# kuleshov-group/PlantCaduceus

Measured on NVIDIA B200. Metric: variants scored/sec, higher is better.
Workload: dtype bf16

## Files before the change

plantcaduceus_b200/csrc/common.cuh:

```cuda
#pragma once

#include <cuda.h>
#include <cuda_bf16.h>
#include <cuda_runtime.h>
#include <stdint.h>

#ifndef __CUDA_ARCH_FEAT_SM100_ALL
#endif

namespace pcad {

typedef __nv_bfloat16 bf16;

template <typename Kernel>
inline cudaError_t ensure_dynamic_smem(Kernel kernel, int bytes, unsigned long long& done) {
  int dev = 0;
  cudaError_t e = cudaGetDevice(&dev);
  if (e != cudaSuccess) return e;
  const unsigned long long bit = 1ull << (dev & 63);
  if (done & bit) return cudaSuccess;
  e = cudaFuncSetAttribute(kernel, cudaFuncAttributeMaxDynamicSharedMemorySize, bytes);
  if (e == cudaSuccess) done |= bit;
  return e;
}

constexpr float kLog2e = 1.4426950408889634f;
constexpr float kLn2 = 0.6931471805599453f;

template <typename T> struct ActT;
template <> struct ActT<bf16> {
  static __device__ __forceinline__ float to_f(bf16 v) { return __bfloat162float(v); }
  static __device__ __forceinline__ bf16 from_f(float v) { return __float2bfloat16_rn(v); }
};
template <> struct ActT<float> {
  static __device__ __forceinline__ float to_f(float v) { return v; }
  static __device__ __forceinline__ float from_f(float v) { return v; }
};

template <typename T> struct Vec16 { static constexpr int N = 16 / sizeof(T); };

template <typename T>
__device__ __forceinline__ void load16(const T* p, float (&out)[16 / sizeof(T)]) {
  uint4 raw = *reinterpret_cast<const uint4*>(p);
  if constexpr (sizeof(T) == 2) {
    const uint32_t w[4] = {raw.x, raw.y, raw.z, raw.w};
#pragma unroll
    for (int i = 0; i < 4; ++i) {
      out[2 * i] = __uint_as_float(w[i] << 16);
      out[2 * i + 1] = __uint_as_float(w[i] & 0xffff0000u);
    }
  } else {
    out[0] = __uint_as_float(raw.x); out[1] = __uint_as_float(raw.y);
    out[2] = __uint_as_float(raw.z); out[3] = __uint_as_float(raw.w);
  }
}

__device__ __forceinline__ uint32_t pack_bf16x2(float lo, float hi) {
  __nv_bfloat162 v = __floats2bfloat162_rn(lo, hi);
  return *reinterpret_cast<uint32_t*>(&v);
}

template <typename T>
__device__ __forceinline__ void store16(T* p, const float (&v)[16 / sizeof(T)]) {
  uint4 raw;
  if constexpr (sizeof(T) == 2) {
    raw.x = pack_bf16x2(v[0], v[1]); raw.y = pack_bf16x2(v[2], v[3]);
    raw.z = pack_bf16x2(v[4], v[5]); raw.w = pack_bf16x2(v[6], v[7]);
  } else {
    raw.x = __float_as_uint(v[0]); raw.y = __float_as_uint(v[1]);
    raw.z = __float_as_uint(v[2]); raw.w = __float_as_uint(v[3]);
  }
  *reinterpret_cast<uint4*>(p) = raw;
}

__device__ __forceinline__ float ex2_approx(float x) {
  float y;
  asm("ex2.approx.ftz.f32 %0, %1;" : "=f"(y) : "f"(x));
  return y;
}
__device__ __forceinline__ float lg2_approx(float x) {
  float y;
  asm("lg2.approx.ftz.f32 %0, %1;" : "=f"(y) : "f"(x));
  return y;
}
__device__ __forceinline__ float rcp_approx(float x) {
  float y;
  asm("rcp.approx.ftz.f32 %0, %1;" : "=f"(y) : "f"(x));
  return y;
}

template <bool PRECISE>
__device__ __forceinline__ float silu(float x) {
  if constexpr (PRECISE) {
    return x / (1.0f + expf(-x));
  } else {
    return x * rcp_approx(1.0f + ex2_approx(-x * kLog2e));
  }
}

template <bool PRECISE>
__device__ __forceinline__ float softplus(float x) {
  if constexpr (PRECISE) {
    return x > 20.0f ? x : log1pf(expf(x));
  } else {
    float sp = lg2_approx(1.0f + ex2_approx(x * kLog2e)) * kLn2;
    return x > 20.0f ? x : sp;
  }
}

typedef unsigned long long f32x2;
__device__ __forceinline__ f32x2 pack2(float lo, float hi) {
  f32x2 r;
  asm("mov.b64 %0, {%1, %2};" : "=l"(r) : "f"(lo), "f"(hi));
  return r;
}
__device__ __forceinline__ void unpack2(f32x2 v, float& lo, float& hi) {
  asm("mov.b64 {%0, %1}, %2;" : "=f"(lo), "=f"(hi) : "l"(v));
}
__device__ __forceinline__ f32x2 fma2(f32x2 a, f32x2 b, f32x2 c) {
  f32x2 r;
  asm("fma.rn.f32x2 %0, %1, %2, %3;" : "=l"(r) : "l"(a), "l"(b), "l"(c));
  return r;
}
__device__ __forceinline__ f32x2 mul2(f32x2 a, f32x2 b) {
  f32x2 r;
  asm("mul.rn.f32x2 %0, %1, %2;" : "=l"(r) : "l"(a), "l"(b));
  return r;
}
__device__ __forceinline__ f32x2 add2(f32x2 a, f32x2 b) {
  f32x2 r;
  asm("add.rn.f32x2 %0, %1, %2;" : "=l"(r) : "l"(a), "l"(b));
  return r;
}

__device__ __forceinline__ f32x2 exp2_poly2(f32x2 x2) {
  float x0, x1;
  unpack2(x2, x0, x1);
  x0 = fmaxf(x0, -126.0f);
  x1 = fmaxf(x1, -126.0f);
  x2 = pack2(x0, x1);
  const f32x2 magic = pack2(12582912.0f, 12582912.0f);
  const f32x2 r2 = add2(x2, magic);
  const f32x2 n2 = add2(r2, pack2(-12582912.0f, -12582912.0f));
  const f32x2 f2 = fma2(n2, pack2(-1.0f, -1.0f), x2);
  f32x2 p = fma2(pack2(0.009582849219441414f, 0.009582849219441414f), f2, pack2(0.05590642988681793f, 0.05590642988681793f));
  p = fma2(p, f2, pack2(0.24024099111557007f, 0.24024099111557007f));
  p = fma2(p, f2, pack2(0.6931241750717163f, 0.6931241750717163f));
  p = fma2(p, f2, pack2(1.0f, 1.0f));
  float p0, p1, r0, r1;
  unpack2(p, p0, p1);
  unpack2(r2, r0, r1);
  p0 = __int_as_float(__float_as_int(p0) + (__float_as_int(r0) << 23));
  p1 = __int_as_float(__float_as_int(p1) + (__float_as_int(r1) << 23));
  return pack2(p0, p1);
}

#ifndef PCAD_POLY_DEG
#define PCAD_POLY_DEG 4
#endif
__device__ __forceinline__ f32x2 exp2_prod_poly2(f32x2 d2, f32x2 a2) {
  const f32x2 magic = pack2(12582912.0f, 12582912.0f);
  const f32x2 r2 = fma2(d2, a2, magic);
  const f32x2 nn2 = fma2(r2, pack2(-1.0f, -1.0f), magic);
  const f32x2 f2 = fma2(d2, a2, nn2);
#if PCAD_POLY_DEG == 3
  f32x2 p = fma2(pack2(0.055009059607982635f, 0.055009059607982635f), f2, pack2(0.2422109693288803f, 0.2422109693288803f));
  p = fma2(p, f2, pack2(0.6932829022407532f, 0.6932829022407532f));
#else
  f32x2 p = fma2(pack2(0.009582576341927052f, 0.009582576341927052f), f2, pack2(0.05590682849287987f, 0.05590682849287987f));
  p = fma2(p, f2, pack2(0.24024106562137604f, 0.24024106562137604f));
  p = fma2(p, f2, pack2(0.6931241154670715f, 0.6931241154670715f));
#endif
  p = fma2(p, f2, pack2(1.0f, 1.0f));
  float p0, p1, r0, r1;
  unpack2(p, p0, p1);
  unpack2(r2, r0, r1);
  p0 = __int_as_float(__float_as_int(p0) + (__float_as_int(r0) << 23));
  p1 = __int_as_float(__float_as_int(p1) + (__float_as_int(r1) << 23));
  return pack2(p0, p1);
}

__device__ __forceinline__ float warp_sum(float v) {
#pragma unroll
  for (int o = 16; o > 0; o >>= 1) v += __shfl_xor_sync(0xffffffffu, v, o);
  return v;
}

__device__ __forceinline__ uint32_t smem_u32(const void* p) {
  return static_cast<uint32_t>(__cvta_generic_to_shared(p));
}

__device__ __forceinline__ void cp_async16(void* smem_dst, const void* gsrc, int src_bytes) {
  asm volatile("cp.async.cg.shared.global [%0], [%1], 16, %2;\n" ::"r"(smem_u32(smem_dst)), "l"(gsrc), "r"(src_bytes));
}
__device__ __forceinline__ void cp_async_commit() { asm volatile("cp.async.commit_group;\n" ::); }
template <int N>
__device__ __forceinline__ void cp_async_wait() { asm volatile("cp.async.wait_group %0;\n" ::"n"(N)); }

__device__ __forceinline__ void mbar_init(uint64_t* bar, uint32_t count) {
  asm volatile("mbarrier.init.shared::cta.b64 [%0], %1;\n" ::"r"(smem_u32(bar)), "r"(count));
}
__device__ __forceinline__ void fence_mbar_init() { asm volatile("fence.mbarrier_init.release.cluster;\n" ::); }
__device__ __forceinline__ void fence_proxy_async_smem() { asm volatile("fence.proxy.async.shared::cta;\n" ::); }

__device__ __forceinline__ void mbar_arrive_expect_tx(uint64_t* bar, uint32_t bytes) {
  asm volatile("mbarrier.arrive.expect_tx.shared::cta.b64 _, [%0], %1;\n" ::"r"(smem_u32(bar)), "r"(bytes) : "memory");
}
__device__ __forceinline__ void mbar_arrive(uint64_t* bar) {
  asm volatile("mbarrier.arrive.shared::cta.b64 _, [%0];\n" ::"r"(smem_u32(bar)) : "memory");
}
__device__ __forceinline__ bool mbar_try_wait(uint64_t* bar, uint32_t parity) {
  uint32_t ok;
  asm volatile(
      "{\n\t.reg .pred P1;\n\t"
      "mbarrier.try_wait.parity.shared::cta.b64 P1, [%1], %2;\n\t"
      "selp.b32 %0, 1, 0, P1;\n\t}\n"
      : "=r"(ok)
      : "r"(smem_u32(bar)), "r"(parity)
      : "memory");
  return ok != 0;
}
__device__ __forceinline__ void mbar_wait(uint64_t* bar, uint32_t parity) {
  while (!mbar_try_wait(bar, parity)) {
  }
}

__device__ __forceinline__ void mbar_wait_or_trap(uint64_t* bar, uint32_t parity) {
  for (uint32_t i = 0; i < (1u << 28); ++i)
    if (mbar_try_wait(bar, parity)) return;
  asm volatile("trap;");
}

__device__ __forceinline__ bool elect_one() {
  uint32_t pred;
  asm volatile(
      "{\n\t.reg .b32 rx;\n\t.reg .pred px;\n\t"
      "elect.sync rx|px, 0xffffffff;\n\t"
      "selp.b32 %0, 1, 0, px;\n\t}\n"
      : "=r"(pred));
  return pred != 0;
}

__device__ __forceinline__ void tma_prefetch_desc(const CUtensorMap* m) {
  asm volatile("prefetch.tensormap [%0];\n" ::"l"(reinterpret_cast<uint64_t>(m)) : "memory");
}
__device__ __forceinline__ void tma_load_2d(void* smem_dst, const CUtensorMap* m, uint64_t* bar, int c0, int c1) {
  asm volatile(
      "cp.async.bulk.tensor.2d.shared::cluster.global.mbarrier::complete_tx::bytes [%0], [%1, {%3, %4}], [%2];\n" ::"r"(
          smem_u32(smem_dst)),
      "l"(reinterpret_cast<uint64_t>(m)), "r"(smem_u32(bar)), "r"(c0), "r"(c1)
      : "memory");
}
__device__ __forceinline__ void tma_load_3d(void* smem_dst, const CUtensorMap* m, uint64_t* bar, int c0, int c1, int c2) {
  asm volatile(
      "cp.async.bulk.tensor.3d.shared::cluster.global.mbarrier::complete_tx::bytes [%0], [%1, {%3, %4, %5}], [%2];\n" ::"r"(
          smem_u32(smem_dst)),
      "l"(reinterpret_cast<uint64_t>(m)), "r"(smem_u32(bar)), "r"(c0), "r"(c1), "r"(c2)
      : "memory");
}
__device__ __forceinline__ void tma_prefetch_l2_3d(const CUtensorMap* m, int c0, int c1, int c2) {
  asm volatile("cp.async.bulk.prefetch.tensor.3d.L2.global [%0, {%1, %2, %3}];\n" ::"l"(reinterpret_cast<uint64_t>(m)), "r"(c0),
               "r"(c1), "r"(c2)
               : "memory");
}
__device__ __forceinline__ void tma_store_2d(const CUtensorMap* m, const void* smem_src, int c0, int c1) {
  asm volatile("cp.async.bulk.tensor.2d.global.shared::cta.bulk_group [%0, {%2, %3}], [%1];\n" ::"l"(
                   reinterpret_cast<uint64_t>(m)),
               "r"(smem_u32(smem_src)), "r"(c0), "r"(c1)
               : "memory");
}
__device__ __forceinline__ void tma_store_commit() { asm volatile("cp.async.bulk.commit_group;\n" ::: "memory"); }
template <int N>
__device__ __forceinline__ void tma_store_wait_read() {
  asm volatile("cp.async.bulk.wait_group.read %0;\n" ::"n"(N) : "memory");
}
template <int N>
__device__ __forceinline__ void tma_store_wait() {
  asm volatile("cp.async.bulk.wait_group %0;\n" ::"n"(N) : "memory");
}

template <int COLS>
__device__ __forceinline__ void tmem_alloc(uint32_t* smem_result) {
  asm volatile("tcgen05.alloc.cta_group::1.sync.aligned.shared::cta.b32 [%0], %1;\n" ::"r"(smem_u32(smem_result)), "n"(COLS)
               : "memory");
}
__device__ __forceinline__ void tmem_relinquish() {
  asm volatile("tcgen05.relinquish_alloc_permit.cta_group::1.sync.aligned;\n" ::: "memory");
}
template <int COLS>
__device__ __forceinline__ void tmem_dealloc(uint32_t taddr) {
  asm volatile("tcgen05.dealloc.cta_group::1.sync.aligned.b32 %0, %1;\n" ::"r"(taddr), "n"(COLS) : "memory");
}
__device__ __forceinline__ void tc_fence_before() { asm volatile("tcgen05.fence::before_thread_sync;\n" ::: "memory"); }
__device__ __forceinline__ void tc_fence_after() { asm volatile("tcgen05.fence::after_thread_sync;\n" ::: "memory"); }

__device__ __forceinline__ void umma_bf16_ss(uint32_t tmem_d, uint64_t desc_a, uint64_t desc_b, uint32_t idesc,
                                             uint32_t accumulate) {
  asm volatile(
      "{\n\t.reg .pred p;\n\t"
      "setp.ne.b32 p, %4, 0;\n\t"
      "tcgen05.mma.cta_group::1.kind::f16 [%0], %1, %2, %3, p;\n\t}\n" ::"r"(tmem_d),
      "l"(desc_a), "l"(desc_b), "r"(idesc), "r"(accumulate)
      : "memory");
}
__device__ __forceinline__ void umma_bf16_ss_k64_commit(uint32_t tmem_d, uint64_t desc_a, uint64_t desc_b, uint32_t idesc,
                                                        int ksteps, uint64_t* bar) {
  asm volatile(
      "{\n\t.reg .pred pz, po, p1, p2, p3;\n\t.reg .b64 a1, b1, a2, b2, a3, b3;\n\t"
      "setp.ne.b32 pz, 0, 0;\n\t"
      "setp.eq.b32 po, 0, 0;\n\t"
      "setp.gt.s32 p1, %4, 1;\n\t"
      "setp.gt.s32 p2, %4, 2;\n\t"
      "setp.gt.s32 p3, %4, 3;\n\t"
      "add.s64 a1, %1, 2;\n\tadd.s64 b1, %2, 2;\n\t"
      "add.s64 a2, %1, 4;\n\tadd.s64 b2, %2, 4;\n\t"
      "add.s64 a3, %1, 6;\n\tadd.s64 b3, %2, 6;\n\t"
      "tcgen05.mma.cta_group::1.kind::f16 [%0], %1, %2, %3, pz;\n\t"
      "@p1 tcgen05.mma.cta_group::1.kind::f16 [%0], a1, b1, %3, po;\n\t"
      "@p2 tcgen05.mma.cta_group::1.kind::f16 [%0], a2, b2, %3, po;\n\t"
      "@p3 tcgen05.mma.cta_group::1.kind::f16 [%0], a3, b3, %3, po;\n\t"
      "tcgen05.commit.cta_group::1.mbarrier::arrive::one.shared::cluster.b64 [%5];\n\t}\n" ::"r"(tmem_d),
      "l"(desc_a), "l"(desc_b), "r"(idesc), "r"(ksteps), "r"(smem_u32(bar))
      : "memory");
}
__device__ __forceinline__ void umma_commit(uint64_t* bar) {
  asm volatile("tcgen05.commit.cta_group::1.mbarrier::arrive::one.shared::cluster.b64 [%0];\n" ::"r"(smem_u32(bar))
               : "memory");
}
__device__ __forceinline__ void tmem_ld_32x32b_x32(uint32_t taddr, uint32_t (&r)[32]) {
  asm volatile(
      "tcgen05.ld.sync.aligned.32x32b.x32.b32 "
      "{%0, %1, %2, %3, %4, %5, %6, %7, %8, %9, %10, %11, %12, %13, %14, %15, "
      "%16, %17, %18, %19, %20, %21, %22, %23, %24, %25, %26, %27, %28, %29, %30, %31}, [%32];\n"
      : "=r"(r[0]), "=r"(r[1]), "=r"(r[2]), "=r"(r[3]), "=r"(r[4]), "=r"(r[5]), "=r"(r[6]), "=r"(r[7]), "=r"(r[8]),
        "=r"(r[9]), "=r"(r[10]), "=r"(r[11]), "=r"(r[12]), "=r"(r[13]), "=r"(r[14]), "=r"(r[15]), "=r"(r[16]),
        "=r"(r[17]), "=r"(r[18]), "=r"(r[19]), "=r"(r[20]), "=r"(r[21]), "=r"(r[22]), "=r"(r[23]), "=r"(r[24]),
        "=r"(r[25]), "=r"(r[26]), "=r"(r[27]), "=r"(r[28]), "=r"(r[29]), "=r"(r[30]), "=r"(r[31])
      : "r"(taddr)
      : "memory");
}
__device__ __forceinline__ void tmem_ld_32x32b_x16(uint32_t taddr, uint32_t (&r)[16]) {
  asm volatile(
      "tcgen05.ld.sync.aligned.32x32b.x16.b32 "
      "{%0, %1, %2, %3, %4, %5, %6, %7, %8, %9, %10, %11, %12, %13, %14, %15}, [%16];\n"
      : "=r"(r[0]), "=r"(r[1]), "=r"(r[2]), "=r"(r[3]), "=r"(r[4]), "=r"(r[5]), "=r"(r[6]), "=r"(r[7]), "=r"(r[8]),
        "=r"(r[9]), "=r"(r[10]), "=r"(r[11]), "=r"(r[12]), "=r"(r[13]), "=r"(r[14]), "=r"(r[15])
      : "r"(taddr)
      : "memory");
}
__device__ __forceinline__ uint32_t tmem_ld_32x32b_x1(uint32_t taddr) {
  uint32_t r;
  asm volatile("tcgen05.ld.sync.aligned.32x32b.x1.b32 {%0}, [%1];\n" : "=r"(r) : "r"(taddr) : "memory");
  return r;
}
__device__ __forceinline__ void tmem_ld_wait() { asm volatile("tcgen05.wait::ld.sync.aligned;\n" ::: "memory"); }

__device__ __forceinline__ uint32_t cluster_ctarank() {
  uint32_t r;
  asm volatile("mov.u32 %0, %%cluster_ctarank;\n" : "=r"(r));
  return r;
}
__device__ __forceinline__ void cluster_sync_all() {
  asm volatile("barrier.cluster.arrive.release.aligned;\n" ::: "memory");
  asm volatile("barrier.cluster.wait.acquire.aligned;\n" ::: "memory");
}
constexpr uint32_t kPeerBitMask = 0xFEFFFFFFu;
__device__ __forceinline__ void tma_load_2d_cg2(void* smem_dst, const CUtensorMap* m, uint64_t* bar, int c0, int c1) {
  asm volatile(
      "cp.async.bulk.tensor.2d.cta_group::2.shared::cluster.global.mbarrier::complete_tx::bytes [%0], [%1, {%3, %4}], [%2];\n" ::"r"(
          smem_u32(smem_dst)),
      "l"(reinterpret_cast<uint64_t>(m)), "r"(smem_u32(bar) & kPeerBitMask), "r"(c0), "r"(c1)
      : "memory");
}
template <int COLS>
__device__ __forceinline__ void tmem_alloc_cg2(uint32_t* smem_result) {
  asm volatile("tcgen05.alloc.cta_group::2.sync.aligned.shared::cta.b32 [%0], %1;\n" ::"r"(smem_u32(smem_result)), "n"(COLS)
               : "memory");
}
__device__ __forceinline__ void tmem_relinquish_cg2() {
  asm volatile("tcgen05.relinquish_alloc_permit.cta_group::2.sync.aligned;\n" ::: "memory");
}
template <int COLS>
__device__ __forceinline__ void tmem_dealloc_cg2(uint32_t taddr) {
  asm volatile("tcgen05.dealloc.cta_group::2.sync.aligned.b32 %0, %1;\n" ::"r"(taddr), "n"(COLS) : "memory");
}
__device__ __forceinline__ void umma_bf16_ss_cg2(uint32_t tmem_d, uint64_t desc_a, uint64_t desc_b, uint32_t idesc,
                                                 uint32_t accumulate) {
  const uint32_t zero = 0;
  asm volatile(
      "{\n\t.reg .pred p;\n\t"
      "setp.ne.b32 p, %4, 0;\n\t"
      "tcgen05.mma.cta_group::2.kind::f16 [%0], %1, %2, %3, {%5, %5, %5, %5, %5, %5, %5, %5}, p;\n\t}\n" ::"r"(tmem_d),
      "l"(desc_a), "l"(desc_b), "r"(idesc), "r"(accumulate), "r"(zero)
      : "memory");
}
__device__ __forceinline__ void umma_commit_cg2(uint64_t* bar) {
  const uint16_t mask = 3;
  asm volatile("tcgen05.commit.cta_group::2.mbarrier::arrive::one.shared::cluster.multicast::cluster.b64 [%0], %1;\n" ::"r"(
                   smem_u32(bar)),
               "h"(mask)
               : "memory");
}
__device__ __forceinline__ void mbar_arrive_leader(uint64_t* bar) {
  asm volatile("mbarrier.arrive.release.cluster.shared::cluster.b64 _, [%0];\n" ::"r"(smem_u32(bar) & kPeerBitMask) : "memory");
}

__device__ __forceinline__ uint64_t make_smem_desc_sw128(uint32_t smem_addr) {
  uint64_t desc = 0;
  desc |= static_cast<uint64_t>((smem_addr & 0x3FFFFu) >> 4);
  desc |= static_cast<uint64_t>(1) << 16;
  desc |= static_cast<uint64_t>(1024 >> 4) << 32;
  desc |= static_cast<uint64_t>(1) << 46;
  desc |= static_cast<uint64_t>(2) << 61;
  return desc;
}

__host__ __device__ constexpr uint32_t make_idesc_bf16(int M, int N) {
  return (1u << 4)
         | (1u << 7)
         | (1u << 10)
         | (0u << 15) | (0u << 16)
         | (static_cast<uint32_t>(N >> 3) << 17)
         | (static_cast<uint32_t>(M >> 4) << 24);
}

typedef CUresult (*PFN_encodeTiled)(CUtensorMap*, CUtensorMapDataType, cuuint32_t, void*, const cuuint64_t*,
                                    const cuuint64_t*, const cuuint32_t*, const cuuint32_t*, CUtensorMapInterleave,
                                    CUtensorMapSwizzle, CUtensorMapL2promotion, CUtensorMapFloatOOBfill);

inline PFN_encodeTiled get_encode_tiled() {
  static PFN_encodeTiled fn = nullptr;
  if (!fn) {
    void* p = nullptr;
    cudaDriverEntryPointQueryResult qres;
    if (cudaGetDriverEntryPoint("cuTensorMapEncodeTiled", &p, cudaEnableDefault, &qres) == cudaSuccess &&
        qres == cudaDriverEntryPointSuccess)
      fn = reinterpret_cast<PFN_encodeTiled>(p);
  }
  return fn;
}


inline bool make_tmap_3d(CUtensorMap* map, bool f32, const void* base, long long n0, long long n1, long long n2,
                         long long ld, int box0, int box1, bool swizzle128 = false) {
  PFN_encodeTiled enc = get_encode_tiled();
  if (!enc) return false;
  const cuuint64_t es = f32 ? 4 : 2;
  cuuint64_t gdim[3] = {static_cast<cuuint64_t>(n0), static_cast<cuuint64_t>(n1), static_cast<cuuint64_t>(n2)};
  cuuint64_t gstride[2] = {static_cast<cuuint64_t>(ld) * es, static_cast<cuuint64_t>(ld) * es * static_cast<cuuint64_t>(n1)};
  cuuint32_t box[3] = {static_cast<cuuint32_t>(box0), static_cast<cuuint32_t>(box1), 1};
  cuuint32_t estr[3] = {1, 1, 1};
  CUresult r = enc(map, f32 ? CU_TENSOR_MAP_DATA_TYPE_FLOAT32 : CU_TENSOR_MAP_DATA_TYPE_BFLOAT16, 3,
                   const_cast<void*>(base), gdim, gstride, box, estr, CU_TENSOR_MAP_INTERLEAVE_NONE,
                   swizzle128 ? CU_TENSOR_MAP_SWIZZLE_128B : CU_TENSOR_MAP_SWIZZLE_NONE, CU_TENSOR_MAP_L2_PROMOTION_L2_256B,
                   CU_TENSOR_MAP_FLOAT_OOB_FILL_NONE);
  return r == CUDA_SUCCESS;
}

}
```

plantcaduceus_b200/csrc/pcad.cu:

```cuda
#include "../../include/pcad.h"

#include <math.h>
#include <stdarg.h>
#include <stdio.h>
#include <stdlib.h>
#include <string.h>

#include <map>
#include <string>
#include <vector>

#include "common.cuh"
#include "elementwise.cuh"
#include "gemm_simt.cuh"
#include "gemm_tcgen05.cuh"
#include "scan.cuh"
#include "ssd.cuh"

using namespace pcad;

namespace {

char g_create_error[512] = "";

struct DirWeights {
  float* conv_w = nullptr;
  float* conv_b = nullptr;
  void* x_proj = nullptr;
  void* dt_proj = nullptr;
  float* dt_bias = nullptr;
  float* A = nullptr;
  float* D = nullptr;
  float* gnorm_w = nullptr;
  bool has[8] = {false, false, false, false, false, false, false, false};
};

struct LayerWeights {
  void* in_proj = nullptr;
  void* in_proj_s = nullptr;
  void* out_proj = nullptr;
  float* norm_w = nullptr;
  DirWeights dir[2];
  bool has_in = false, has_out = false, has_norm = false;
};

struct Workspace {
  int B = 0, L = 0;
  size_t bytes = 0;
  uint8_t* base = nullptr;
  uint8_t* ids = nullptr;
  void* hid = nullptr;
  void* resid = nullptr;
  void* normed = nullptr;
  void* xz = nullptr;
  void* xc[2] = {nullptr, nullptr};
  void* dbc[2] = {nullptr, nullptr};
  void* delta[2] = {nullptr, nullptr};
  void* y = nullptr;
  float* sumsq[2] = {nullptr, nullptr};
  float* seg_state = nullptr;
  float* seg_sumd = nullptr;
  float* bcf = nullptr;
  uint8_t* ascii = nullptr;
  float* logits4 = nullptr;
  int* pos = nullptr;
  int* pos0 = nullptr;
};

}

struct pcad_handle {
  pcad_config cfg;
  int device = 0;
  int num_sms = 148;
  int d = 0, E = 0, N = 16, R = 0, RP = 0, V = 8;
  bool m2 = false;
  int ssd_impl = 0;
  int H = 0, CD = 0, DIP = 0, DIPP = 0;
  bool f32 = false;
  bool fuse_dt = false;
  bool bc_f32 = true;
  bool bc_f32_force = false;
  bool fuse_norm = false;
  size_t act_size = 2;
  bool finalized = false;
  char err[512] = "";
  std::vector<LayerWeights> layers;
  void* emb = nullptr;
  float* head_w = nullptr;
  float* norm_f = nullptr;
  bool has_emb = false, has_head = false, has_norm_f = false;
  uint8_t* comp_dev = nullptr;
  uint8_t* lut_dev = nullptr;
  int* sel_dev = nullptr;
  int* bad_flag = nullptr;
  volatile int* bad_flag_host = nullptr;
  int mask_id = 1;
  int acgt[4] = {3, 4, 5, 6};
  Workspace ws;
  std::vector<void*> allocs;
  struct ScoreGraph { int B, L, token_idx; bool seen_only; cudaGraphExec_t exec; int64_t launches; };
  std::vector<ScoreGraph> graphs;
  bool prune_last = true;
  bool last_pruned = false;
  bool time_parallel = true;
  bool use_graphs = true;
  cudaStream_t gstream = nullptr;
  cudaEvent_t g_in = nullptr, g_out = nullptr;
  long long graph_max_tokens = 65536;
  bool profiling = false;
  std::vector<std::pair<int, std::pair<cudaEvent_t, cudaEvent_t>>> prof_events;
  std::vector<cudaEvent_t> event_pool;
  float prof_ms[PCAD_ST_COUNT];
  int64_t prof_launches[PCAD_ST_COUNT];
  int64_t launch_count = 0;
};

namespace {

int fail(pcad_handle* h, int code, const char* fmt, ...) {
  va_list ap;
  va_start(ap, fmt);
  char* dst = h ? h->err : g_create_error;
  vsnprintf(dst, 512, fmt, ap);
  va_end(ap);
  return code;
}

#define CUDA_TRY(h, expr)                                                                          \
  do {                                                                                             \
    cudaError_t _e = (expr);                                                                       \
    if (_e != cudaSuccess)                                                                         \
      return fail((h), PCAD_ERR_CUDA, "%s failed: %s (%s:%d)", #expr, cudaGetErrorString(_e), __FILE__, __LINE__); \
  } while (0)

template <typename T>
int dev_alloc(pcad_handle* h, T** p, size_t count) {
  void* q = nullptr;
  cudaError_t e = cudaMalloc(&q, count * sizeof(T) > 0 ? count * sizeof(T) : 16);
  if (e != cudaSuccess) return fail(h, PCAD_ERR_NOMEM, "cudaMalloc(%zu) failed: %s", count * sizeof(T), cudaGetErrorString(e));
  h->allocs.push_back(q);
  *p = static_cast<T*>(q);
  return PCAD_OK;
}

template <typename SrcT, typename DstT>
__global__ void convert_kernel(const SrcT* __restrict__ src, DstT* __restrict__ dst, long long n) {
  const long long i = static_cast<long long>(blockIdx.x) * blockDim.x + threadIdx.x;
  if (i >= n) return;
  float v;
  if constexpr (sizeof(SrcT) == 2) v = __bfloat162float(src[i]); else v = src[i];
  if constexpr (sizeof(DstT) == 2) dst[i] = __float2bfloat16_rn(v); else dst[i] = v;
}
__global__ void half_to_float_kernel(const __half* __restrict__ src, float* __restrict__ dst, long long n) {
  const long long i = static_cast<long long>(blockIdx.x) * blockDim.x + threadIdx.x;
  if (i < n) dst[i] = __half2float(src[i]);
}
__global__ void scale_columns_kernel(const bf16* __restrict__ W, const float* __restrict__ w, bf16* __restrict__ out,
                                     long long rows, int cols) {
  const long long i = static_cast<long long>(blockIdx.x) * blockDim.x + threadIdx.x;
  if (i >= rows * cols) return;
  out[i] = __float2bfloat16_rn(__bfloat162float(W[i]) * w[i % cols]);
}
__global__ void row_sumsq_kernel(const bf16* __restrict__ x, float* __restrict__ ss, long long rows, int d, int parts) {
  const int lane = threadIdx.x & 31;
  const long long row = static_cast<long long>(blockIdx.x) * (blockDim.x >> 5) + (threadIdx.x >> 5);
  if (row >= rows) return;
  float acc = 0.f;
  for (int j = lane * 8; j < d; j += 256) {
    float v[8];
    load16<bf16>(x + row * d + j, v);
#pragma unroll
    for (int k = 0; k < 8; ++k) acc = fmaf(v[k], v[k], acc);
  }
  acc = warp_sum(acc);
  if (lane < parts) ss[row * parts + lane] = lane == 0 ? acc : 0.f;
}
__global__ void neg_exp_kernel(float* __restrict__ a, long long n) {
  const long long i = static_cast<long long>(blockIdx.x) * blockDim.x + threadIdx.x;
  if (i < n) a[i] = -expf(a[i]);
}

int ingest(pcad_handle* h, const void* src, int src_dtype, void* dst, bool dst_f32, long long n) {
  const size_t src_size = (src_dtype == PCAD_F32) ? 4 : 2;
  void* stage = nullptr;
  CUDA_TRY(h, cudaMalloc(&stage, n * src_size));
  cudaError_t e = cudaMemcpy(stage, src, n * src_size, cudaMemcpyDefault);
  if (e != cudaSuccess) { cudaFree(stage); return fail(h, PCAD_ERR_CUDA, "weight copy failed: %s", cudaGetErrorString(e)); }
  float* f32_tmp = nullptr;
  const void* s = stage;
  int s_dtype = src_dtype;
  const int threads = 256;
  const unsigned blocks = static_cast<unsigned>((n + threads - 1) / threads);
  if (src_dtype == PCAD_F16) {
    e = cudaMalloc(reinterpret_cast<void**>(&f32_tmp), n * 4);
    if (e != cudaSuccess) { cudaFree(stage); return fail(h, PCAD_ERR_NOMEM, "cudaMalloc failed"); }
    half_to_float_kernel<<<blocks, threads>>>(static_cast<const __half*>(stage), f32_tmp, n);
    s = f32_tmp;
    s_dtype = PCAD_F32;
  }
  if (s_dtype == PCAD_F32) {
    if (dst_f32) convert_kernel<float, float><<<blocks, threads>>>(static_cast<const float*>(s), static_cast<float*>(dst), n);
    else convert_kernel<float, bf16><<<blocks, threads>>>(static_cast<const float*>(s), static_cast<bf16*>(dst), n);
  } else {
    if (dst_f32) convert_kernel<bf16, float><<<blocks, threads>>>(static_cast<const bf16*>(s), static_cast<float*>(dst), n);
    else convert_kernel<bf16, bf16><<<blocks, threads>>>(static_cast<const bf16*>(s), static_cast<bf16*>(dst), n);
  }
  e = cudaDeviceSynchronize();
  cudaFree(stage);
  if (f32_tmp) cudaFree(f32_tmp);
  if (e != cudaSuccess) return fail(h, PCAD_ERR_CUDA, "weight conversion failed: %s", cudaGetErrorString(e));
  return PCAD_OK;
}

bool shape_is(const int64_t* shape, int ndim, std::initializer_list<int64_t> want) {
  std::vector<int64_t> a, b;
  for (int i = 0; i < ndim; ++i) if (shape[i] != 1) a.push_back(shape[i]);
  for (int64_t w : want) if (w != 1) b.push_back(w);
  return a == b;
}

struct StageTimer {
  pcad_handle* h;
  cudaStream_t st;
  int stage;
  cudaEvent_t a = nullptr, b = nullptr;
  StageTimer(pcad_handle* h_, cudaStream_t st_, int stage_, int launches = 1) : h(h_), st(st_), stage(stage_) {
    h->launch_count += launches;
    if (!h->profiling) return;
    h->prof_launches[stage] += launches;
    auto get = [&]() {
      cudaEvent_t ev;
      if (!h->event_pool.empty()) { ev = h->event_pool.back(); h->event_pool.pop_back(); }
      else cudaEventCreate(&ev);
      return ev;
    };
    a = get(); b = get();
    cudaEventRecord(a, st);
  }
  ~StageTimer() {
    if (!a) return;
    cudaEventRecord(b, st);
    h->prof_events.push_back({stage, {a, b}});
  }
};

bool gemm_cta_pair_enabled() {
  static int v = -1;
  if (v < 0) {
    const char* e = getenv("PCAD_GEMM_2CTA");
    v = (e && e[0] == '0') ? 0 : 1;
  }
  return v == 1;
}

int op_linear(pcad_handle* h, const void* A, const void* W, void* C, long long M, int N, int K, long long lda,
              long long ldw, long long ldc, bool f32, int num_sms, cudaStream_t st, int epi = kEpiPlain,
              const EpiParams& ep = EpiParams()) {
  if (f32) {
    if (epi != kEpiPlain) return fail(h, PCAD_ERR_INVALID, "fused GEMM epilogues exist for bf16 only");
    CUDA_TRY(h, gemm_f32_simt(static_cast<const float*>(A), static_cast<const float*>(W), static_cast<float*>(C), M, N, K, lda, ldw, ldc, st));
  } else {
    const char* why = nullptr;
    cudaError_t e = gemm_bf16_tcgen05(static_cast<const bf16*>(A), static_cast<const bf16*>(W), static_cast<bf16*>(C), M, N, K, lda, ldw, ldc, num_sms, st, &why, epi, ep, gemm_cta_pair_enabled());
    if (e != cudaSuccess) return fail(h, why ? PCAD_ERR_INVALID : PCAD_ERR_CUDA, "%s", why ? why : cudaGetErrorString(e));
  }
  return PCAD_OK;
}

template <typename T, typename RT>
int launch_norm_t(pcad_handle* h, const void* x, const void* res_in, const float* w, void* y, void* res_out,
                  long long rows, int d, float eps, cudaStream_t st) {
  const int nvec = d / 8;
  const int ch = (nvec + 31) / 32;
  const int warps = 8;
  const unsigned blocks = static_cast<unsigned>((rows + warps - 1) / warps);
#define NORM_CASE(CHV)                                                                                          \
  add_rmsnorm_kernel<T, RT, CHV><<<blocks, warps * 32, 0, st>>>(static_cast<const T*>(x), static_cast<const RT*>(res_in), w, \
                                                               static_cast<T*>(y), static_cast<RT*>(res_out), rows, d, eps)
  if (ch <= 1) NORM_CASE(1);
  else if (ch <= 2) NORM_CASE(2);
  else if (ch <= 4) NORM_CASE(4);
  else if (ch <= 8) NORM_CASE(8);
  else return fail(h, PCAD_ERR_INVALID, "add_rmsnorm: d=%d too large (max 2048)", d);
#undef NORM_CASE
  CUDA_TRY(h, cudaGetLastError());
  return PCAD_OK;
}

int op_add_rmsnorm(pcad_handle* h, const void* x, const void* res_in, const float* w, void* y, void* res_out,
                   long long rows, int d, float eps, bool f32, bool res_f32, cudaStream_t st) {
  if (d % 8) return fail(h, PCAD_ERR_INVALID, "add_rmsnorm: d must be a multiple of 8");
  if (rows <= 0) return PCAD_OK;
  if (f32) return launch_norm_t<float, float>(h, x, res_in, w, y, res_out, rows, d, eps, st);
  if (res_f32) return launch_norm_t<bf16, float>(h, x, res_in, w, y, res_out, rows, d, eps, st);
  return launch_norm_t<bf16, bf16>(h, x, res_in, w, y, res_out, rows, d, eps, st);
}

int op_conv(pcad_handle* h, const void* x, long long ldx, const float* w_f, const float* b_f, const float* w_r,
            const float* b_r, void* out_f, void* out_r, int S, int L, int E, bool f32, cudaStream_t st) {
  if (E % 4) return fail(h, PCAD_ERR_INVALID, "conv: E must be a multiple of 4");
  if (S <= 0 || L <= 0) return PCAD_OK;
  const int cpt = f32 ? 4 : 2;
  dim3 grid((E / cpt + 127) / 128, (L + kConvTT - 1) / kConvTT, S);
  if (f32) conv_silu_kernel<float, true, 4><<<grid, 128, 0, st>>>(static_cast<const float*>(x), ldx, w_f, b_f, w_r, b_r, static_cast<float*>(out_f), static_cast<float*>(out_r), L, E);
  else conv_silu_kernel<bf16, false, 2><<<grid, 128, 0, st>>>(static_cast<const bf16*>(x), ldx, w_f, b_f, w_r, b_r, static_cast<bf16*>(out_f), static_cast<bf16*>(out_r), L, E);
  CUDA_TRY(h, cudaGetLastError());
  return PCAD_OK;
}

int op_biscan(pcad_handle* h, const void* u_f, const void* delta_f, const void* bc_f, const void* u_r,
              const void* delta_r, const void* bc_r, long long ldbc, int bc_off, const void* z, long long ldz,
              const float* A_f, const float* D_f, const float* bias_f, const float* A_r, const float* D_r,
              const float* bias_r, void* y, int S, int L, int E, bool f32, cudaStream_t st,
              const void* wdt_f = nullptr, const void* wdt_r = nullptr, long long ldw = 0, int R = 0, int segments = 1,
              float* seg_state = nullptr, float* seg_sumd = nullptr, int Lrun = 0, float* bcf = nullptr) {
  const int vec = f32 ? 4 : 8;
  if (E % vec || ldbc % vec || bc_off % vec || ldz % vec)
    return fail(h, PCAD_ERR_INVALID, "biscan: E, ldbc, bc_off, ldz must be multiples of %d elements", vec);
  if (S <= 0 || L <= 0) return PCAD_OK;
  if (S > 65535) return fail(h, PCAD_ERR_INVALID, "biscan: at most 65535 sequences per call");
  cudaError_t e;
#define PCAD_SCAN_ARGS(TT)                                                                                           \
  static_cast<const TT*>(u_f), static_cast<const TT*>(delta_f), static_cast<const TT*>(bc_f), static_cast<const TT*>(u_r), \
      static_cast<const TT*>(delta_r), static_cast<const TT*>(bc_r), ldbc, bc_off, static_cast<const TT*>(z), ldz, A_f, D_f, \
      bias_f, A_r, D_r, bias_r, static_cast<TT*>(y), S, L, E
  const bool fused_dt = wdt_f != nullptr || wdt_r != nullptr;
  const float* bcf_f = nullptr;
  const float* bcf_r = nullptr;
  if (bcf && !f32 && !fused_dt) {
    const long long rows = static_cast<long long>(S) * L;
    bc_to_f32_kernel<<<static_cast<unsigned>((rows * 8 + 255) / 256), 256, 0, st>>>(static_cast<const bf16*>(bc_f), static_cast<const bf16*>(bc_r),
                                                                                  ldbc, bc_off, bcf, rows);
    CUDA_TRY(h, cudaGetLastError());
    bcf_f = bcf;
    bcf_r = bcf + rows * 2 * kScanN;
  }
  if (segments > 1) {
    if (fused_dt || !seg_state || !seg_sumd || L % segments || static_cast<long long>(S) * segments > 65535)
      return fail(h, PCAD_ERR_INVALID, "biscan: the time-parallel scan needs L %% segments == 0, S * segments <= 65535 and its state buffers");
    if (f32) e = launch_biscan_time_parallel<float, true>(PCAD_SCAN_ARGS(float), segments, seg_state, seg_sumd, st);
    else e = launch_biscan_time_parallel<bf16, false>(PCAD_SCAN_ARGS(bf16), segments, seg_state, seg_sumd, st, bcf_f, bcf_r);
    CUDA_TRY(h, e);
    return PCAD_OK;
  }
  if (fused_dt) {
    if (f32 || !wdt_f || !wdt_r || ldbc < kScanDtK || R <= 0 || R > kScanDtK || ldw < R || ldw % 8)
      return fail(h, PCAD_ERR_INVALID, "biscan: the in-kernel dt_proj needs bf16, both weights (R <= 64, row pitch a multiple of 8) and ldbc >= 64");
    e = launch_biscan<bf16, false, kScanFusedDt>(PCAD_SCAN_ARGS(bf16), st, static_cast<const bf16*>(wdt_f), static_cast<const bf16*>(wdt_r),
                                                 ldw, R, nullptr, Lrun);
  } else if (f32) {
    e = launch_biscan<float, true, kScanPlain>(PCAD_SCAN_ARGS(float), st, nullptr, nullptr, 0, 0, nullptr, Lrun);
  } else if (bcf_f) {
    e = launch_biscan<bf16, false, kScanBcF32>(PCAD_SCAN_ARGS(bf16), st, nullptr, nullptr, 0, 0, nullptr, Lrun, bcf_f, bcf_r);
  } else {
    e = launch_biscan<bf16, false, kScanPlain>(PCAD_SCAN_ARGS(bf16), st, nullptr, nullptr, 0, 0, nullptr, Lrun);
  }
#undef PCAD_SCAN_ARGS
  CUDA_TRY(h, e);
  return PCAD_OK;
}

size_t align_up(size_t v, size_t a) { return (v + a - 1) / a * a; }
constexpr size_t kSegStateBytes = 16u << 20;

size_t workspace_layout(const pcad_handle* h, int B, int L, Workspace* ws) {
  const size_t T = 2ull * B * L;
  const size_t a = h->act_size;
  const size_t rs = h->f32 ? 4 : (h->cfg.residual_in_fp32 ? 4 : 2);
  size_t off = 0;
  auto take = [&](size_t bytes) { size_t o = off; off = align_up(off + bytes, 1024); return o; };
  const size_t o_ids = take(static_cast<size_t>(B) * L);
  const size_t o_hid = take(T * h->d * a);
  const size_t o_res = take(T * h->d * rs);
  const size_t o_nrm = take(T * h->d * a);
  const size_t w_xz = h->m2 ? h->DIPP : 2 * h->E, w_xc = h->m2 ? h->CD : h->E, w_dbc = h->m2 ? 0 : h->RP;
  const size_t o_xz = take(T * w_xz * a);
  const size_t o_xc0 = take(T * w_xc * a), o_xc1 = take(T * w_xc * a);
  const size_t o_dbc0 = take(T * w_dbc * a), o_dbc1 = take(T * w_dbc * a);
  const size_t o_dl0 = take(T * h->E * a), o_dl1 = take(T * h->E * a);
  const size_t o_y = take(T * h->E * a);
  const size_t ss_parts = static_cast<size_t>(gemm_sumsq_parts(h->d));
  const size_t o_ss0 = take(T * ss_parts * sizeof(float)), o_ss1 = take(T * ss_parts * sizeof(float));
  const size_t o_segs = take(h->m2 ? 0 : kSegStateBytes), o_segd = take(h->m2 ? 0 : kSegStateBytes / 16);
  const size_t o_bcf = take((h->m2 || h->f32) ? 0 : T * 2 * 2 * kScanN * sizeof(float));
  const size_t o_ascii = take(static_cast<size_t>(B) * L);
  const size_t o_l4 = take(static_cast<size_t>(B) * 4 * sizeof(float));
  const size_t o_pos = take(static_cast<size_t>(B) * sizeof(int));
  const size_t o_pos0 = take(static_cast<size_t>(B) * sizeof(int));
  if (ws && ws->base) {
    uint8_t* p = ws->base;
    ws->ids = p + o_ids; ws->hid = p + o_hid; ws->resid = p + o_res; ws->normed = p + o_nrm; ws->xz = p + o_xz;
    ws->xc[0] = p + o_xc0; ws->xc[1] = p + o_xc1; ws->dbc[0] = p + o_dbc0; ws->dbc[1] = p + o_dbc1;
    ws->delta[0] = p + o_dl0; ws->delta[1] = p + o_dl1; ws->y = p + o_y;
    ws->sumsq[0] = reinterpret_cast<float*>(p + o_ss0); ws->sumsq[1] = reinterpret_cast<float*>(p + o_ss1);
    ws->seg_state = reinterpret_cast<float*>(p + o_segs); ws->seg_sumd = reinterpret_cast<float*>(p + o_segd);
    ws->bcf = (h->m2 || h->f32) ? nullptr : reinterpret_cast<float*>(p + o_bcf);
    ws->ascii = p + o_ascii; ws->logits4 = reinterpret_cast<float*>(p + o_l4); ws->pos = reinterpret_cast<int*>(p + o_pos);
    ws->pos0 = reinterpret_cast<int*>(p + o_pos0);
  }
  return off;
}

void clear_graphs(pcad_handle* h) {
  for (auto& g : h->graphs)
    if (g.exec) cudaGraphExecDestroy(g.exec);
  h->graphs.clear();
}

int ensure_workspace(pcad_handle* h, int B, int L) {
  Workspace& ws = h->ws;
  const size_t need = workspace_layout(h, B, L, nullptr);
  if (ws.base == nullptr || need > ws.bytes) {
    clear_graphs(h);
    if (ws.base) { cudaDeviceSynchronize(); cudaFree(ws.base); ws.base = nullptr; ws.bytes = 0; }
    void* p = nullptr;
    cudaError_t e = cudaMalloc(&p, need);
    if (e != cudaSuccess) return fail(h, PCAD_ERR_NOMEM, "workspace cudaMalloc(%zu bytes) for B=%d L=%d failed: %s", need, B, L, cudaGetErrorString(e));
    ws.base = static_cast<uint8_t*>(p);
    ws.bytes = need;
  }
  ws.B = B; ws.L = L;
  workspace_layout(h, B, L, &ws);
  return PCAD_OK;
}

int op_ssd_scan(pcad_handle* h, const void* xbc_f, const void* xbc_r, long long ld_xbc, const void* dt_raw, long long ld_dt,
                const float* A_f, const float* D_f, const float* bias_f, const float* A_r, const float* D_r, const float* bias_r,
                void* y_f, void* y_r, int S, int L, int H, bool f32, int impl, cudaStream_t st) {
  const bool sequential = impl == 1;
  if (S <= 0 || L <= 0) return PCAD_OK;
  if (H <= 0 || S > 65535) return fail(h, PCAD_ERR_INVALID, "ssd_scan: need H > 0 and at most 65535 sequences per call");
  cudaError_t e;
  if (f32) {
    e = launch_ssd_seq<float>(static_cast<const float*>(xbc_f), static_cast<const float*>(xbc_r), ld_xbc, static_cast<const float*>(dt_raw),
                              ld_dt, A_f, D_f, bias_f, A_r, D_r, bias_r, static_cast<float*>(y_f), static_cast<float*>(y_r), S, L, H, st);
  } else if (sequential) {
    e = launch_ssd_seq<bf16>(static_cast<const bf16*>(xbc_f), static_cast<const bf16*>(xbc_r), ld_xbc, static_cast<const bf16*>(dt_raw),
                             ld_dt, A_f, D_f, bias_f, A_r, D_r, bias_r, static_cast<bf16*>(y_f), static_cast<bf16*>(y_r), S, L, H, st);
  } else {
    if ((H & 1) || (ld_xbc % 8) || (reinterpret_cast<uintptr_t>(xbc_f) & 15) || (reinterpret_cast<uintptr_t>(xbc_r) & 15) ||
        (reinterpret_cast<uintptr_t>(y_f) & 15) || (reinterpret_cast<uintptr_t>(y_r) & 15))
      return fail(h, PCAD_ERR_INVALID, "ssd_scan: the tensor-core kernel needs an even head count, 16-byte aligned tensors and ld_xbc %% 8 == 0");
    e = launch_ssd_tc(static_cast<const bf16*>(xbc_f), static_cast<const bf16*>(xbc_r), ld_xbc, static_cast<const bf16*>(dt_raw), ld_dt,
                      A_f, D_f, bias_f, A_r, D_r, bias_r, static_cast<bf16*>(y_f), static_cast<bf16*>(y_r), S, L, H, st);
  }
  CUDA_TRY(h, e);
  return PCAD_OK;
}

int op_gated_norm_sum(pcad_handle* h, const void* y_f, const void* y_r, const void* z, long long ldz, const float* w_f,
                      const float* w_r, void* out, long long rows, int E, float eps, bool f32, cudaStream_t st) {
  if (rows <= 0) return PCAD_OK;
  const int vec = f32 ? 4 : 8;
  if (E % vec || ldz % vec) return fail(h, PCAD_ERR_INVALID, "gated_norm_sum: E and ldz must be multiples of %d", vec);
  const unsigned blocks = static_cast<unsigned>((rows + 7) / 8);
  if (!f32 && E <= 256 * 12) {
    const int ch = (E + 255) / 256;
#define GN_CASE(CHV)                                                                                                        \
  gated_norm_sum_regs_kernel<CHV><<<blocks, 256, 0, st>>>(static_cast<const bf16*>(y_f), static_cast<const bf16*>(y_r),        \
                                                          static_cast<const bf16*>(z), ldz, w_f, w_r, static_cast<bf16*>(out), rows, E, eps)
    if (ch <= 1) GN_CASE(1);
    else if (ch <= 2) GN_CASE(2);
    else if (ch <= 3) GN_CASE(3);
    else if (ch <= 4) GN_CASE(4);
    else if (ch <= 6) GN_CASE(6);
    else if (ch <= 8) GN_CASE(8);
    else GN_CASE(12);
#undef GN_CASE
    CUDA_TRY(h, cudaGetLastError());
    return PCAD_OK;
  }
  if (f32) gated_norm_sum_kernel<float, true><<<blocks, 256, 0, st>>>(static_cast<const float*>(y_f), static_cast<const float*>(y_r), static_cast<const float*>(z), ldz, w_f, w_r, static_cast<float*>(out), rows, E, eps);
  else gated_norm_sum_kernel<bf16, false><<<blocks, 256, 0, st>>>(static_cast<const bf16*>(y_f), static_cast<const bf16*>(y_r), static_cast<const bf16*>(z), ldz, w_f, w_r, static_cast<bf16*>(out), rows, E, eps);
  CUDA_TRY(h, cudaGetLastError());
  return PCAD_OK;
}

int run_mixer_m2(pcad_handle* h, LayerWeights& lw, int S, int L, cudaStream_t st) {
  Workspace& ws = h->ws;
  const long long T = static_cast<long long>(S) * L;
  const int E = h->E, CD = h->CD, H = h->H;
  const bool f32 = h->f32;
  const size_t a = h->act_size;
  uint8_t* zx = static_cast<uint8_t*>(ws.xz);
  int rc;
  {
    StageTimer tm(h, st, PCAD_ST_CONV);
    rc = op_conv(h, zx + static_cast<size_t>(E) * a, h->DIPP, lw.dir[0].conv_w, lw.dir[0].conv_b, lw.dir[1].conv_w, lw.dir[1].conv_b,
                 ws.xc[0], ws.xc[1], S, L, CD, f32, st);
    if (rc) return rc;
  }
  {
    StageTimer tm(h, st, PCAD_ST_SCAN);
    rc = op_ssd_scan(h, ws.xc[0], ws.xc[1], CD, zx + static_cast<size_t>(E + CD) * a, h->DIPP, lw.dir[0].A, lw.dir[0].D, lw.dir[0].dt_bias,
                     lw.dir[1].A, lw.dir[1].D, lw.dir[1].dt_bias, ws.delta[0], ws.delta[1], S, L, H, f32, h->ssd_impl, st);
    if (rc) return rc;
  }
  {
    StageTimer tm(h, st, PCAD_ST_GNORM);
    rc = op_gated_norm_sum(h, ws.delta[0], ws.delta[1], zx, h->DIPP, lw.dir[0].gnorm_w, lw.dir[1].gnorm_w, ws.y, T, E, 1e-5f, f32, st);
    if (rc) return rc;
  }
  return PCAD_OK;
}

__global__ void gather_rows_kernel(const uint4* __restrict__ src, uint4* __restrict__ dst, int S, int B, int L, int idx, int vec_per_row) {
  const long long gid = static_cast<long long>(blockIdx.x) * blockDim.x + threadIdx.x;
  if (gid >= static_cast<long long>(S) * vec_per_row) return;
  const int s = static_cast<int>(gid / vec_per_row), v = static_cast<int>(gid % vec_per_row);
  const int row = s < B ? idx : L - 1 - idx;
  dst[gid] = src[(static_cast<long long>(s) * L + row) * vec_per_row + v];
}

int run_backbone(pcad_handle* h, int B, int L, cudaStream_t st, int prune_idx = -1) {
  Workspace& ws = h->ws;
  const long long T = 2LL * B * L;
  const int S = 2 * B;
  const int d = h->d, E = h->E, R = h->R, RP = h->RP;
  const bool f32 = h->f32;
  const bool res_f32 = f32 || h->cfg.residual_in_fp32;
  const bool fused = h->fuse_norm;
  int cur = 0;
  h->last_pruned = false;
  const int parts = gemm_sumsq_parts(d);
  const int n_in = h->m2 ? h->DIP : 2 * E;
  const long long ld_in = h->m2 ? h->DIPP : 2 * E;
  {
    StageTimer tm(h, st, PCAD_ST_EMBED, fused ? 2 : 1);
    const long long total = T * (d / 8);
    const unsigned blocks = static_cast<unsigned>((total + 255) / 256);
    if (f32) embed_kernel<float><<<blocks, 256, 0, st>>>(ws.ids, static_cast<const float*>(h->emb), static_cast<float*>(ws.hid), B, L, d, h->comp_dev);
    else embed_kernel<bf16><<<blocks, 256, 0, st>>>(ws.ids, static_cast<const bf16*>(h->emb), static_cast<bf16*>(fused ? ws.resid : ws.hid), B, L, d, h->comp_dev);
    if (fused) row_sumsq_kernel<<<static_cast<unsigned>((T + 7) / 8), 256, 0, st>>>(static_cast<const bf16*>(ws.resid), ws.sumsq[cur], T, d, parts);
    CUDA_TRY(h, cudaGetLastError());
  }
  for (int li = 0; li < h->cfg.n_layer; ++li) {
    LayerWeights& lw = h->layers[li];
    int rc;
    bool pruned = false;
    if (!fused) {
      StageTimer tm(h, st, PCAD_ST_NORM);
      rc = op_add_rmsnorm(h, ws.hid, li == 0 ? nullptr : ws.resid, lw.norm_w, ws.normed, ws.resid, T, d, h->cfg.norm_eps, f32, res_f32, st);
      if (rc) return rc;
    }
    {
      StageTimer tm(h, st, PCAD_ST_IN_PROJ);
      if (fused) {
        EpiParams ep;
        ep.sumsq_in = ws.sumsq[cur];
        ep.sumsq_parts = parts;
        ep.inv_k = 1.0f / static_cast<float>(d);
        ep.eps = h->cfg.norm_eps;
        rc = op_linear(h, ws.resid, lw.in_proj_s, ws.xz, T, n_in, d, d, d, ld_in, false, h->num_sms, st, kEpiRowScale, ep);
      } else {
        rc = op_linear(h, ws.normed, lw.in_proj, ws.xz, T, n_in, d, d, d, ld_in, f32, h->num_sms, st);
      }
      if (rc) return rc;
    }
    if (h->m2) {
      rc = run_mixer_m2(h, lw, S, L, st);
      if (rc) return rc;
    } else {
    {
      StageTimer tm(h, st, PCAD_ST_CONV);
      rc = op_conv(h, ws.xz, 2 * E, lw.dir[0].conv_w, lw.dir[0].conv_b, lw.dir[1].conv_w, lw.dir[1].conv_b, ws.xc[0], ws.xc[1], S, L, E, f32, st);
      if (rc) return rc;
    }
    int P = 1;
    if (h->time_parallel) {
      const long long ctas = static_cast<long long>((E + kScanCH - 1) / kScanCH) * S, slots = 4LL * h->num_sms;
      while (P < 32 && ctas * P * 2 <= slots && L % (P * 2) == 0 && L / (P * 2) >= 512 &&
             static_cast<size_t>(S) * P * 2 * 2 * E * kScanN * sizeof(float) <= kSegStateBytes)
        P *= 2;
    }
    const bool fuse_dt = h->fuse_dt && P == 1;
    for (int dir = 0; dir < 2; ++dir) {
      {
        StageTimer tm(h, st, PCAD_ST_X_PROJ);
        rc = op_linear(h, ws.xc[dir], lw.dir[dir].x_proj, ws.dbc[dir], T, RP, E, E, E, RP, f32, h->num_sms, st);
        if (rc) return rc;
      }
      if (!fuse_dt) {
        StageTimer tm(h, st, PCAD_ST_DT_PROJ);
        rc = op_linear(h, ws.dbc[dir], lw.dir[dir].dt_proj, ws.delta[dir], T, E, R, RP, R, E, f32, h->num_sms, st);
        if (rc) return rc;
      }
    }
    {
      StageTimer tm(h, st, PCAD_ST_SCAN);
      const uint8_t* zbase = static_cast<const uint8_t*>(ws.xz) + static_cast<size_t>(E) * h->act_size;
      pruned = prune_idx >= 0 && li == h->cfg.n_layer - 1 && P == 1 && h->prune_last && L >= 8;
      const int Lrun = pruned ? (prune_idx > L - 1 - prune_idx ? prune_idx : L - 1 - prune_idx) + 1 : 0;
      const bool use_bcf = h->bc_f32 && !f32 && (h->bc_f32_force || T >= 65536);
      if (fuse_dt)
        rc = op_biscan(h, ws.xc[0], ws.dbc[0], ws.dbc[0], ws.xc[1], ws.dbc[1], ws.dbc[1], RP, R, zbase, 2 * E,
                       lw.dir[0].A, lw.dir[0].D, lw.dir[0].dt_bias, lw.dir[1].A, lw.dir[1].D, lw.dir[1].dt_bias, ws.y, S, L, E, f32,
                       st, lw.dir[0].dt_proj, lw.dir[1].dt_proj, R, R, 1, nullptr, nullptr, Lrun);
      else {
        rc = op_biscan(h, ws.xc[0], ws.delta[0], ws.dbc[0], ws.xc[1], ws.delta[1], ws.dbc[1], RP, R, zbase, 2 * E,
                       lw.dir[0].A, lw.dir[0].D, lw.dir[0].dt_bias, lw.dir[1].A, lw.dir[1].D, lw.dir[1].dt_bias, ws.y, S, L, E, f32, st,
                       nullptr, nullptr, 0, 0, P, ws.seg_state, ws.seg_sumd, Lrun, use_bcf ? ws.bcf : nullptr);
        if (P > 1) h->launch_count += 2;
        if (use_bcf) h->launch_count += 1;
      }
      if (rc) return rc;
    }
    }
    if (pruned) {
      h->last_pruned = true;
      const size_t a = h->act_size, rs = res_f32 ? 4 : a;
      uint8_t* yc = static_cast<uint8_t*>(ws.delta[0]);
      uint8_t* rc_in = static_cast<uint8_t*>(ws.delta[1]);
      uint8_t* rc_out = rc_in + align_up(static_cast<size_t>(S) * d * 4, 1024);
      {
        StageTimer tm(h, st, PCAD_ST_MISC, 2);
        const int vy = static_cast<int>(E * a / 16), vr = static_cast<int>(d * rs / 16);
        gather_rows_kernel<<<static_cast<unsigned>((static_cast<long long>(S) * vy + 255) / 256), 256, 0, st>>>(
            static_cast<const uint4*>(ws.y), reinterpret_cast<uint4*>(yc), S, B, L, prune_idx, vy);
        if (fused || li > 0)
          gather_rows_kernel<<<static_cast<unsigned>((static_cast<long long>(S) * vr + 255) / 256), 256, 0, st>>>(
              static_cast<const uint4*>(ws.resid), reinterpret_cast<uint4*>(rc_in), S, B, L, prune_idx, vr);
        CUDA_TRY(h, cudaGetLastError());
      }
      {
        StageTimer tm(h, st, PCAD_ST_OUT_PROJ);
        if (fused) {
          EpiParams ep;
          ep.resid = reinterpret_cast<const bf16*>(rc_in);
          ep.ld_res = d;
          ep.sumsq_out = ws.sumsq[cur ^ 1];
          ep.sumsq_parts = parts;
          rc = op_linear(h, yc, lw.out_proj, rc_out, S, d, E, E, E, d, false, h->num_sms, st, kEpiResidual, ep);
        } else {
          rc = op_linear(h, yc, lw.out_proj, rc_out, S, d, E, E, E, d, f32, h->num_sms, st);
        }
        if (rc) return rc;
      }
      StageTimer tm(h, st, PCAD_ST_NORM);
      if (fused) rc = op_add_rmsnorm(h, rc_out, nullptr, h->norm_f, ws.normed, nullptr, S, d, h->cfg.norm_eps, false, false, st);
      else rc = op_add_rmsnorm(h, rc_out, li == 0 ? nullptr : rc_in, h->norm_f, ws.normed, nullptr, S, d, h->cfg.norm_eps, f32, res_f32, st);
      return rc;
    }
    {
      StageTimer tm(h, st, PCAD_ST_OUT_PROJ);
      if (fused) {
        EpiParams ep;
        ep.resid = static_cast<const bf16*>(ws.resid);
        ep.ld_res = d;
        ep.sumsq_out = ws.sumsq[cur ^ 1];
        ep.sumsq_parts = parts;
        rc = op_linear(h, ws.y, lw.out_proj, ws.resid, T, d, E, E, E, d, false, h->num_sms, st, kEpiResidual, ep);
        cur ^= 1;
      } else {
        rc = op_linear(h, ws.y, lw.out_proj, ws.hid, T, d, E, E, E, d, f32, h->num_sms, st);
      }
      if (rc) return rc;
    }
  }
  {
    StageTimer tm(h, st, PCAD_ST_NORM);
    int rc;
    if (fused) rc = op_add_rmsnorm(h, ws.resid, nullptr, h->norm_f, ws.normed, nullptr, T, d, h->cfg.norm_eps, false, false, st);
    else rc = op_add_rmsnorm(h, ws.hid, h->cfg.n_layer == 0 ? nullptr : ws.resid, h->norm_f, ws.normed, nullptr, T, d, h->cfg.norm_eps, f32, res_f32, st);
    if (rc) return rc;
  }
  return PCAD_OK;
}

int run_head(pcad_handle* h, int B, int L, const int* pos_dev, int n_pos, float* out, cudaStream_t st) {
  StageTimer tm(h, st, PCAD_ST_HEAD);
  const long long items = pos_dev ? static_cast<long long>(B) * n_pos : static_cast<long long>(B) * L;
  if (items <= 0) return PCAD_OK;
  const unsigned blocks = static_cast<unsigned>((items + 7) / 8);
  if (h->f32) lm_head_kernel<float><<<blocks, 256, 0, st>>>(static_cast<const float*>(h->ws.normed), h->head_w, h->comp_dev, pos_dev, n_pos, h->sel_dev, out, B, L, h->d);
  else lm_head_kernel<bf16><<<blocks, 256, 0, st>>>(static_cast<const bf16*>(h->ws.normed), h->head_w, h->comp_dev, pos_dev, n_pos, h->sel_dev, out, B, L, h->d);
  CUDA_TRY(h, cudaGetLastError());
  return PCAD_OK;
}

__global__ void fill_int_kernel(int* p, int n, int v) {
  const int i = blockIdx.x * blockDim.x + threadIdx.x;
  if (i < n) p[i] = v;
}

int check_call(pcad_handle* h, int B, int L) {
  if (!h) return PCAD_ERR_INVALID;
  if (!h->finalized) return fail(h, PCAD_ERR_STATE, "pcad_finalize must succeed before a forward call");
  if (B < 0 || L < 0) return fail(h, PCAD_ERR_INVALID, "negative batch or length");
  if (2LL * B > 65535) return fail(h, PCAD_ERR_INVALID, "B=%d too large for one call (max 32767)", B);
  return PCAD_OK;
}

}

extern "C" {

int pcad_abi_version(void) { return PCAD_ABI_VERSION; }

const char* pcad_last_error(const pcad_handle* h) { return h ? h->err : g_create_error; }

int pcad_create(const pcad_config* cfg, int device, pcad_handle** out) {
  if (!cfg || !out) return fail(nullptr, PCAD_ERR_INVALID, "null argument");
  *out = nullptr;
  const bool m2 = cfg->mixer == PCAD_MIXER_MAMBA2;
  if (cfg->mixer != PCAD_MIXER_MAMBA1 && !m2) return fail(nullptr, PCAD_ERR_INVALID, "unknown mixer %d", cfg->mixer);
  if (m2) {
    if (cfg->d_state != 64 || cfg->headdim != 64 || cfg->ngroups != 1)
      return fail(nullptr, PCAD_ERR_INVALID, "unsupported Mamba-2 shape d_state=%d headdim=%d ngroups=%d (engine is specialised for 64 / 64 / 1)",
                  cfg->d_state, cfg->headdim, cfg->ngroups);
    if ((cfg->expand * cfg->d_model / 64) % 2) return fail(nullptr, PCAD_ERR_INVALID, "Mamba-2 needs an even number of heads");
  } else if (cfg->d_state != 16) {
    return fail(nullptr, PCAD_ERR_INVALID, "unsupported d_state=%d (engine is specialised for 16)", cfg->d_state);
  }
  if (cfg->d_conv != 4) return fail(nullptr, PCAD_ERR_INVALID, "unsupported d_conv=%d (engine is specialised for 4)", cfg->d_conv);
  if (cfg->vocab_size != 8) return fail(nullptr, PCAD_ERR_INVALID, "unsupported vocab_size=%d (LM head is specialised for 8 rows)", cfg->vocab_size);
  if (cfg->d_model <= 0 || cfg->d_model % 128 != 0 || cfg->d_model > 2048)
    return fail(nullptr, PCAD_ERR_INVALID, "unsupported d_model=%d (need a multiple of 128, <= 2048)", cfg->d_model);
  if (cfg->expand != 2) return fail(nullptr, PCAD_ERR_INVALID, "unsupported expand=%d", cfg->expand);
  if (!m2 && (cfg->dt_rank <= 0 || cfg->dt_rank % 8 != 0)) return fail(nullptr, PCAD_ERR_INVALID, "unsupported dt_rank=%d (need a multiple of 8)", cfg->dt_rank);
  if (cfg->n_layer < 0) return fail(nullptr, PCAD_ERR_INVALID, "negative n_layer");
  if (cfg->dtype != PCAD_BF16 && cfg->dtype != PCAD_F32) return fail(nullptr, PCAD_ERR_INVALID, "dtype must be PCAD_BF16 or PCAD_F32");
  for (int i = 0; i < cfg->vocab_size; ++i)
    if (cfg->complement_map[i] < 0 || cfg->complement_map[i] >= cfg->vocab_size)
      return fail(nullptr, PCAD_ERR_INVALID, "complement_map[%d]=%d out of range", i, cfg->complement_map[i]);
  int ndev = 0;
  cudaError_t e = cudaGetDeviceCount(&ndev);
  if (e != cudaSuccess || ndev == 0)
    return fail(nullptr, PCAD_ERR_CUDA, "no CUDA device available (%s); libpcad has no CPU fallback", cudaGetErrorString(e));
  if (device < 0 || device >= ndev) return fail(nullptr, PCAD_ERR_INVALID, "device %d out of range (have %d)", device, ndev);
  e = cudaSetDevice(device);
  if (e != cudaSuccess) return fail(nullptr, PCAD_ERR_CUDA, "cudaSetDevice failed: %s", cudaGetErrorString(e));
  cudaDeviceProp prop;
  cudaGetDeviceProperties(&prop, device);
  if (prop.major != 10)
    return fail(nullptr, PCAD_ERR_CUDA, "device %d is sm_%d%d; libpcad is built for sm_100a only", device, prop.major, prop.minor);

  pcad_handle* h = new pcad_handle();
  h->cfg = *cfg;
  h->device = device;
  h->num_sms = prop.multiProcessorCount;
  h->d = cfg->d_model;
  h->E = cfg->expand * cfg->d_model;
  h->N = cfg->d_state;
  h->R = cfg->dt_rank;
  h->RP = (h->R + 2 * h->N + 15) / 16 * 16;
  h->m2 = m2;
  if (m2) {
    h->H = h->E / 64;
    h->CD = h->E + 2 * h->N;
    h->DIP = h->E + h->CD + h->H;
    h->DIPP = (h->DIP + 7) / 8 * 8;
    h->R = 0;
    h->RP = 0;
    if (const char* sq = getenv("PCAD_SSD_SEQ")) h->ssd_impl = sq[0] == '1' ? 1 : 0;
  }
  h->V = cfg->vocab_size;
  h->f32 = cfg->dtype == PCAD_F32;
  h->act_size = h->f32 ? 4 : 2;
  h->fuse_norm = !h->f32 && !cfg->residual_in_fp32;
  h->fuse_dt = false;
  if (const char* fd = getenv("PCAD_FUSED_DT"))
    h->fuse_dt = fd[0] == '1' && !m2 && !h->f32 && h->RP >= kScanDtK && h->R <= kScanDtK && (h->E % 8) == 0;
  if (const char* bq = getenv("PCAD_SCAN_BC_F32")) { h->bc_f32 = bq[0] != '0'; h->bc_f32_force = bq[0] == '1'; }
  if (const char* pl = getenv("PCAD_NO_PRUNE")) h->prune_last = pl[0] != '1';
  if (const char* tp = getenv("PCAD_NO_TIME_PARALLEL")) h->time_parallel = tp[0] != '1';
  if (const char* ng = getenv("PCAD_NO_GRAPH")) h->use_graphs = ng[0] != '1';
  if (const char* gm = getenv("PCAD_GRAPH_MAX_TOKENS")) h->graph_max_tokens = atoll(gm);
  if (const char* nf = getenv("PCAD_NO_FUSED_NORM")) { if (nf[0] == '1') h->fuse_norm = false; }
  memset(h->prof_ms, 0, sizeof(h->prof_ms));
  memset(h->prof_launches, 0, sizeof(h->prof_launches));
  h->layers.resize(cfg->n_layer);
  int rc = PCAD_OK;
  const size_t a = h->act_size;
  auto A8 = [&](void** p, size_t bytes) { uint8_t* q; int r = dev_alloc<uint8_t>(h, &q, bytes); *p = q; return r; };
  rc |= A8(&h->emb, static_cast<size_t>(h->V) * h->d * a);
  rc |= dev_alloc(h, &h->head_w, static_cast<size_t>(h->V) * h->d);
  rc |= dev_alloc(h, &h->norm_f, h->d);
  rc |= dev_alloc(h, &h->comp_dev, 16);
  rc |= dev_alloc(h, &h->lut_dev, 256);
  rc |= dev_alloc(h, &h->sel_dev, 4);
  {
    void* hp = nullptr;
    void* dp = nullptr;
    if (cudaHostAlloc(&hp, sizeof(int), cudaHostAllocMapped) != cudaSuccess || cudaHostGetDevicePointer(&dp, hp, 0) != cudaSuccess) {
      if (hp) cudaFreeHost(hp);
      rc |= fail(h, PCAD_ERR_NOMEM, "cudaHostAlloc for the id-error flag failed");
    } else {
      h->bad_flag_host = static_cast<volatile int*>(hp);
      *h->bad_flag_host = 0;
      h->bad_flag = static_cast<int*>(dp);
    }
  }
  const size_t n_in_rows = m2 ? static_cast<size_t>(h->DIP) : static_cast<size_t>(2) * h->E;
  for (auto& lw : h->layers) {
    rc |= A8(&lw.in_proj, n_in_rows * h->d * a);
    if (h->fuse_norm) rc |= A8(&lw.in_proj_s, n_in_rows * h->d * a);
    rc |= A8(&lw.out_proj, static_cast<size_t>(h->d) * h->E * a);
    rc |= dev_alloc(h, &lw.norm_w, h->d);
    for (int dir = 0; dir < 2; ++dir) {
      DirWeights& dw = lw.dir[dir];
      if (m2) {
        rc |= dev_alloc(h, &dw.conv_w, static_cast<size_t>(h->CD) * 4);
        rc |= dev_alloc(h, &dw.conv_b, h->CD);
        rc |= dev_alloc(h, &dw.dt_bias, h->H);
        rc |= dev_alloc(h, &dw.A, h->H);
        rc |= dev_alloc(h, &dw.D, h->H);
        rc |= dev_alloc(h, &dw.gnorm_w, h->E);
        continue;
      }
      rc |= dev_alloc(h, &dw.conv_w, static_cast<size_t>(h->E) * 4);
      rc |= dev_alloc(h, &dw.conv_b, h->E);
      rc |= A8(&dw.x_proj, static_cast<size_t>(h->RP) * h->E * a);
      rc |= A8(&dw.dt_proj, static_cast<size_t>(h->E) * h->R * a);
      rc |= dev_alloc(h, &dw.dt_bias, h->E);
      rc |= dev_alloc(h, &dw.A, static_cast<size_t>(h->E) * h->N);
      rc |= dev_alloc(h, &dw.D, h->E);
      if (rc == PCAD_OK) cudaMemset(dw.x_proj, 0, static_cast<size_t>(h->RP) * h->E * a);
    }
    if (rc != PCAD_OK) break;
  }
  if (rc != PCAD_OK) {
    snprintf(g_create_error, sizeof(g_create_error), "%.511s", h->err);
    pcad_destroy(h);
    return PCAD_ERR_NOMEM;
  }
  uint8_t comp8[16] = {0};
  for (int i = 0; i < h->V; ++i) comp8[i] = static_cast<uint8_t>(cfg->complement_map[i]);
  cudaMemcpy(h->comp_dev, comp8, 16, cudaMemcpyHostToDevice);
  uint8_t lut[256];
  memset(lut, 2, sizeof(lut));
  lut['a'] = lut['A'] = 3; lut['c'] = lut['C'] = 4; lut['g'] = lut['G'] = 5; lut['t'] = lut['T'] = 6;
  const int32_t acgt[4] = {3, 4, 5, 6};
  *out = h;
  return pcad_set_tokenizer(h, lut, 1, acgt);
}

void pcad_destroy(pcad_handle* h) {
  if (!h) return;
  cudaSetDevice(h->device);
  cudaDeviceSynchronize();
  for (auto& pe : h->prof_events) { cudaEventDestroy(pe.second.first); cudaEventDestroy(pe.second.second); }
  for (auto ev : h->event_pool) cudaEventDestroy(ev);
  clear_graphs(h);
  if (h->gstream) cudaStreamDestroy(h->gstream);
  if (h->g_in) cudaEventDestroy(h->g_in);
  if (h->g_out) cudaEventDestroy(h->g_out);
  if (h->ws.base) cudaFree(h->ws.base);
  if (h->bad_flag_host) cudaFreeHost(const_cast<int*>(h->bad_flag_host));
  for (void* p : h->allocs) cudaFree(p);
  delete h;
}

int pcad_set_tokenizer(pcad_handle* h, const uint8_t lut[256], int mask_id, const int32_t acgt_ids[4]) {
  if (!h || !lut || !acgt_ids) return PCAD_ERR_INVALID;
  if (mask_id < 0 || mask_id >= h->V) return fail(h, PCAD_ERR_INVALID, "mask_id %d out of range", mask_id);
  for (int i = 0; i < 256; ++i) if (lut[i] >= h->V) return fail(h, PCAD_ERR_INVALID, "lut[%d]=%d out of range", i, lut[i]);
  for (int k = 0; k < 4; ++k) if (acgt_ids[k] < 0 || acgt_ids[k] >= h->V) return fail(h, PCAD_ERR_INVALID, "acgt id out of range");
  CUDA_TRY(h, cudaSetDevice(h->device));
  CUDA_TRY(h, cudaMemcpy(h->lut_dev, lut, 256, cudaMemcpyHostToDevice));
  int sel[4] = {acgt_ids[0], acgt_ids[1], acgt_ids[2], acgt_ids[3]};
  CUDA_TRY(h, cudaMemcpy(h->sel_dev, sel, sizeof(sel), cudaMemcpyHostToDevice));
  h->mask_id = mask_id;
  for (int k = 0; k < 4; ++k) h->acgt[k] = acgt_ids[k];
  clear_graphs(h);
  return PCAD_OK;
}

int pcad_set_weight(pcad_handle* h, const char* name, const void* data, const int64_t* shape, int ndim, int src_dtype) {
  if (!h || !name || !data || !shape) return PCAD_ERR_INVALID;
  if (src_dtype != PCAD_BF16 && src_dtype != PCAD_F32 && src_dtype != PCAD_F16) return fail(h, PCAD_ERR_INVALID, "bad src_dtype for %s", name);
  CUDA_TRY(h, cudaSetDevice(h->device));
  h->finalized = false;
  clear_graphs(h);
  const int d = h->d, E = h->E, N = h->N, R = h->R, V = h->V;
  const std::string s(name);
  auto bad_shape = [&]() { return fail(h, PCAD_ERR_INVALID, "unexpected shape for %s", name); };
  if (s == "caduceus.backbone.embeddings.word_embeddings.embedding.weight") {
    if (!shape_is(shape, ndim, {V, d})) return bad_shape();
    int rc = ingest(h, data, src_dtype, h->emb, h->f32, static_cast<long long>(V) * d);
    h->has_emb = rc == PCAD_OK;
    return rc;
  }
  if (s == "lm_head.lm_head.weight") {
    if (!shape_is(shape, ndim, {V, d})) return bad_shape();
    int rc = ingest(h, data, src_dtype, h->head_w, true, static_cast<long long>(V) * d);
    h->has_head = rc == PCAD_OK;
    return rc;
  }
  if (s == "caduceus.backbone.norm_f.weight") {
    if (!shape_is(shape, ndim, {d})) return bad_shape();
    int rc = ingest(h, data, src_dtype, h->norm_f, true, d);
    h->has_norm_f = rc == PCAD_OK;
    return rc;
  }
  const std::string lp = "caduceus.backbone.layers.";
  if (s.compare(0, lp.size(), lp) != 0) return fail(h, PCAD_ERR_INVALID, "unknown weight name %s", name);
  size_t dot = s.find('.', lp.size());
  if (dot == std::string::npos) return fail(h, PCAD_ERR_INVALID, "unknown weight name %s", name);
  const int li = atoi(s.substr(lp.size(), dot - lp.size()).c_str());
  if (li < 0 || li >= h->cfg.n_layer) return fail(h, PCAD_ERR_INVALID, "layer index out of range in %s", name);
  LayerWeights& lw = h->layers[li];
  const std::string rest = s.substr(dot + 1);
  if (rest == "norm.weight") {
    if (!shape_is(shape, ndim, {d})) return bad_shape();
    int rc = ingest(h, data, src_dtype, lw.norm_w, true, d);
    lw.has_norm = rc == PCAD_OK;
    return rc;
  }
  const std::string mp = "mixer.submodule.mamba_";
  if (rest.compare(0, mp.size(), mp) != 0) return fail(h, PCAD_ERR_INVALID, "unknown weight name %s", name);
  int dir;
  if (rest.compare(mp.size(), 4, "fwd.") == 0) dir = 0;
  else if (rest.compare(mp.size(), 4, "rev.") == 0) dir = 1;
  else return fail(h, PCAD_ERR_INVALID, "unknown weight name %s", name);
  const std::string leaf = rest.substr(mp.size() + 4);
  DirWeights& dw = lw.dir[dir];
  int rc;
  const int n_in = h->m2 ? h->DIP : 2 * E;
  const int CE = h->m2 ? h->CD : E;
  const int NH = h->m2 ? h->H : E;
  if (leaf == "in_proj.weight") {
    if (!shape_is(shape, ndim, {n_in, d})) return bad_shape();
    if (dir == 1 && lw.has_in) return PCAD_OK;
    rc = ingest(h, data, src_dtype, lw.in_proj, h->f32, static_cast<long long>(n_in) * d);
    lw.has_in = rc == PCAD_OK;
  } else if (leaf == "out_proj.weight") {
    if (!shape_is(shape, ndim, {d, E})) return bad_shape();
    if (dir == 1 && lw.has_out) return PCAD_OK;
    rc = ingest(h, data, src_dtype, lw.out_proj, h->f32, static_cast<long long>(d) * E);
    lw.has_out = rc == PCAD_OK;
  } else if (leaf == "conv1d.weight") {
    if (!shape_is(shape, ndim, {CE, 4})) return bad_shape();
    rc = ingest(h, data, src_dtype, dw.conv_w, true, static_cast<long long>(CE) * 4);
    dw.has[0] = rc == PCAD_OK;
  } else if (leaf == "conv1d.bias") {
    if (!shape_is(shape, ndim, {CE})) return bad_shape();
    rc = ingest(h, data, src_dtype, dw.conv_b, true, CE);
    dw.has[1] = rc == PCAD_OK;
  } else if (leaf == "x_proj.weight" && !h->m2) {
    if (!shape_is(shape, ndim, {R + 2 * N, E})) return bad_shape();
    rc = ingest(h, data, src_dtype, dw.x_proj, h->f32, static_cast<long long>(R + 2 * N) * E);
    dw.has[2] = rc == PCAD_OK;
  } else if (leaf == "dt_proj.weight" && !h->m2) {
    if (!shape_is(shape, ndim, {E, R})) return bad_shape();
    rc = ingest(h, data, src_dtype, dw.dt_proj, h->f32, static_cast<long long>(E) * R);
    dw.has[3] = rc == PCAD_OK;
  } else if ((leaf == "dt_proj.bias" && !h->m2) || (leaf == "dt_bias" && h->m2)) {
    if (!shape_is(shape, ndim, {NH})) return bad_shape();
    rc = ingest(h, data, src_dtype, dw.dt_bias, true, NH);
    dw.has[4] = rc == PCAD_OK;
  } else if (leaf == "A_log") {
    const long long n = h->m2 ? NH : static_cast<long long>(E) * N;
    if (h->m2 ? !shape_is(shape, ndim, {NH}) : !shape_is(shape, ndim, {E, N})) return bad_shape();
    rc = ingest(h, data, src_dtype, dw.A, true, n);
    if (rc == PCAD_OK) {
      neg_exp_kernel<<<static_cast<unsigned>((n + 255) / 256), 256>>>(dw.A, n);
      CUDA_TRY(h, cudaDeviceSynchronize());
    }
    dw.has[5] = rc == PCAD_OK;
  } else if (leaf == "D") {
    if (!shape_is(shape, ndim, {NH})) return bad_shape();
    rc = ingest(h, data, src_dtype, dw.D, true, NH);
    dw.has[6] = rc == PCAD_OK;
  } else if (leaf == "norm.weight" && h->m2) {
    if (!shape_is(shape, ndim, {E})) return bad_shape();
    rc = ingest(h, data, src_dtype, dw.gnorm_w, true, E);
    dw.has[7] = rc == PCAD_OK;
  } else {
    return fail(h, PCAD_ERR_INVALID, "unknown weight name %s", name);
  }
  return rc;
}

int pcad_finalize(pcad_handle* h) {
  if (!h) return PCAD_ERR_INVALID;
  if (!h->has_emb) return fail(h, PCAD_ERR_MISSING, "missing weight: embedding");
  if (!h->has_norm_f) return fail(h, PCAD_ERR_MISSING, "missing weight: norm_f");
  if (!h->has_head) {
    const long long n = static_cast<long long>(h->V) * h->d;
    CUDA_TRY(h, cudaSetDevice(h->device));
    if (h->f32) convert_kernel<float, float><<<static_cast<unsigned>((n + 255) / 256), 256>>>(static_cast<const float*>(h->emb), h->head_w, n);
    else convert_kernel<bf16, float><<<static_cast<unsigned>((n + 255) / 256), 256>>>(static_cast<const bf16*>(h->emb), h->head_w, n);
    CUDA_TRY(h, cudaDeviceSynchronize());
    h->has_head = true;
  }
  static const char* names1[8] = {"conv1d.weight", "conv1d.bias", "x_proj.weight", "dt_proj.weight", "dt_proj.bias", "A_log", "D", nullptr};
  static const char* names2[8] = {"conv1d.weight", "conv1d.bias", nullptr, nullptr, "dt_bias", "A_log", "D", "norm.weight"};
  const char** names = h->m2 ? names2 : names1;
  for (int li = 0; li < h->cfg.n_layer; ++li) {
    const LayerWeights& lw = h->layers[li];
    if (!lw.has_in) return fail(h, PCAD_ERR_MISSING, "missing weight: layers.%d in_proj.weight", li);
    if (!lw.has_out) return fail(h, PCAD_ERR_MISSING, "missing weight: layers.%d out_proj.weight", li);
    if (!lw.has_norm) return fail(h, PCAD_ERR_MISSING, "missing weight: layers.%d norm.weight", li);
    for (int dir = 0; dir < 2; ++dir)
      for (int k = 0; k < 8; ++k)
        if (names[k] && !lw.dir[dir].has[k]) return fail(h, PCAD_ERR_MISSING, "missing weight: layers.%d mamba_%s.%s", li, dir ? "rev" : "fwd", names[k]);
  }
  if (h->fuse_norm) {
    CUDA_TRY(h, cudaSetDevice(h->device));
    const long long rows = h->m2 ? h->DIP : 2LL * h->E, n = rows * h->d;
    for (auto& lw : h->layers)
      scale_columns_kernel<<<static_cast<unsigned>((n + 255) / 256), 256>>>(static_cast<const bf16*>(lw.in_proj), lw.norm_w,
                                                                           static_cast<bf16*>(lw.in_proj_s), rows, h->d);
    CUDA_TRY(h, cudaDeviceSynchronize());
  }
  h->finalized = true;
  return PCAD_OK;
}

int pcad_workspace_bytes(pcad_handle* h, int B, int L, size_t* out) {
  if (!h || !out || B < 0 || L < 0) return PCAD_ERR_INVALID;
  *out = workspace_layout(h, B, L, nullptr);
  return PCAD_OK;
}

int pcad_tokenize(pcad_handle* h, const uint8_t* ascii_dev, int64_t n, uint8_t* ids_dev, void* stream) {
  if (!h || (n > 0 && (!ascii_dev || !ids_dev))) return PCAD_ERR_INVALID;
  if (n <= 0) return PCAD_OK;
  CUDA_TRY(h, cudaSetDevice(h->device));
  cudaStream_t st = static_cast<cudaStream_t>(stream);
  StageTimer tm(h, st, PCAD_ST_MISC);
  tokenize_kernel<<<static_cast<unsigned>((n + 255) / 256), 256, 0, st>>>(ascii_dev, ids_dev, n, h->lut_dev, 1, -1, 0);
  CUDA_TRY(h, cudaGetLastError());
  return PCAD_OK;
}

int pcad_extract_windows(pcad_handle* h, const uint8_t* chrom_dev, int64_t chrom_len, const int64_t* pos0_dev, int B, int L,
                         int token_idx, uint8_t* ascii_out_dev, void* stream) {
  if (!h || B < 0 || L <= 0 || chrom_len < 0) return PCAD_ERR_INVALID;
  if (B == 0) return PCAD_OK;
  if (!chrom_dev || !pos0_dev || !ascii_out_dev) return fail(h, PCAD_ERR_INVALID, "null argument");
  if (token_idx < 0 || token_idx >= L) return fail(h, PCAD_ERR_INVALID, "token_idx %d outside [0, %d)", token_idx, L);
  CUDA_TRY(h, cudaSetDevice(h->device));
  cudaStream_t st = static_cast<cudaStream_t>(stream);
  StageTimer tm(h, st, PCAD_ST_MISC);
  const long long n = static_cast<long long>(B) * L;
  extract_windows_kernel<<<static_cast<unsigned>((n + 255) / 256), 256, 0, st>>>(
      chrom_dev, chrom_len, reinterpret_cast<const long long*>(pos0_dev), ascii_out_dev, B, L, token_idx);
  CUDA_TRY(h, cudaGetLastError());
  return PCAD_OK;
}

namespace {
int score_core(pcad_handle* h, int B, int L, int token_idx, cudaStream_t st) {
  Workspace& ws = h->ws;
  const long long n = static_cast<long long>(B) * L;
  {
    StageTimer tm(h, st, PCAD_ST_MISC, 3);
    tokenize_kernel<<<static_cast<unsigned>((n + 255) / 256), 256, 0, st>>>(ws.ascii, ws.ids, n, h->lut_dev, L, token_idx, h->mask_id);
    fill_int_kernel<<<(B + 255) / 256, 256, 0, st>>>(ws.pos, B, token_idx);
    fill_int_kernel<<<(B + 255) / 256, 256, 0, st>>>(ws.pos0, B, 0);
    CUDA_TRY(h, cudaGetLastError());
  }
  const bool prune = h->prune_last && !h->m2 && h->cfg.n_layer > 0;
  int rc = run_backbone(h, B, L, st, prune ? token_idx : -1);
  if (rc) return rc;
  if (prune && h->last_pruned) return run_head(h, B, 1, ws.pos0, 1, ws.logits4, st);
  return run_head(h, B, L, ws.pos, 1, ws.logits4, st);
}

int score_core_graphed(pcad_handle* h, int B, int L, int token_idx, cudaStream_t st) {
  if (!h->use_graphs || h->profiling || 2LL * B * L > h->graph_max_tokens) return score_core(h, B, L, token_idx, st);
  pcad_handle::ScoreGraph* e = nullptr;
  for (auto& g : h->graphs)
    if (g.B == B && g.L == L && g.token_idx == token_idx) { e = &g; break; }
  if (!e) {
    h->graphs.push_back({B, L, token_idx, true, nullptr, 0});
    return score_core(h, B, L, token_idx, st);
  }
  if (!h->gstream) {
    if (cudaStreamCreateWithFlags(&h->gstream, cudaStreamNonBlocking) != cudaSuccess ||
        cudaEventCreateWithFlags(&h->g_in, cudaEventDisableTiming) != cudaSuccess ||
        cudaEventCreateWithFlags(&h->g_out, cudaEventDisableTiming) != cudaSuccess) {
      h->use_graphs = false;
      cudaGetLastError();
      return score_core(h, B, L, token_idx, st);
    }
  }
  if (e->seen_only) {
    const int64_t before = h->launch_count;
    cudaGraph_t graph = nullptr;
    cudaError_t ce = cudaStreamBeginCapture(h->gstream, cudaStreamCaptureModeThreadLocal);
    int rc = ce == cudaSuccess ? score_core(h, B, L, token_idx, h->gstream) : PCAD_ERR_CUDA;
    if (ce == cudaSuccess) ce = cudaStreamEndCapture(h->gstream, &graph);
    if (rc == PCAD_OK && ce == cudaSuccess && graph) ce = cudaGraphInstantiate(&e->exec, graph, 0);
    if (graph) cudaGraphDestroy(graph);
    if (rc != PCAD_OK || ce != cudaSuccess || !e->exec) {
      e->exec = nullptr;
      h->use_graphs = false;
      h->launch_count = before;
      cudaGetLastError();
      return score_core(h, B, L, token_idx, st);
    }
    e->launches = h->launch_count - before;
    h->launch_count = before;
    e->seen_only = false;
  }
  CUDA_TRY(h, cudaEventRecord(h->g_in, st));
  CUDA_TRY(h, cudaStreamWaitEvent(h->gstream, h->g_in, 0));
  CUDA_TRY(h, cudaGraphLaunch(e->exec, h->gstream));
  CUDA_TRY(h, cudaEventRecord(h->g_out, h->gstream));
  CUDA_TRY(h, cudaStreamWaitEvent(st, h->g_out, 0));
  h->launch_count += e->launches;
  return PCAD_OK;
}
}

int pcad_score_windows_dev(pcad_handle* h, const uint8_t* ascii_dev, int B, int L, int token_idx, float* logits4_dev, void* stream) {
  int rc = check_call(h, B, L);
  if (rc) return rc;
  if (B == 0 || L == 0) return PCAD_OK;
  if (!ascii_dev || !logits4_dev) return fail(h, PCAD_ERR_INVALID, "null argument");
  if (token_idx < 0 || token_idx >= L) return fail(h, PCAD_ERR_INVALID, "token_idx %d outside [0, %d)", token_idx, L);
  CUDA_TRY(h, cudaSetDevice(h->device));
  cudaStream_t st = static_cast<cudaStream_t>(stream);
  rc = ensure_workspace(h, B, L);
  if (rc) return rc;
  Workspace& ws = h->ws;
  const size_t n = static_cast<size_t>(B) * L;
  CUDA_TRY(h, cudaMemcpyAsync(ws.ascii, ascii_dev, n, cudaMemcpyDeviceToDevice, st));
  rc = score_core_graphed(h, B, L, token_idx, st);
  if (rc) return rc;
  CUDA_TRY(h, cudaMemcpyAsync(logits4_dev, ws.logits4, static_cast<size_t>(B) * 4 * sizeof(float), cudaMemcpyDeviceToDevice, st));
  return PCAD_OK;
}

int pcad_forward(pcad_handle* h, const int64_t* ids_dev, int B, int L, float* logits_dev, void* hidden_dev, void* stream) {
  int rc = check_call(h, B, L);
  if (rc) return rc;
  if (B == 0 || L == 0) return PCAD_OK;
  if (!ids_dev) return fail(h, PCAD_ERR_INVALID, "ids_dev is null");
  CUDA_TRY(h, cudaSetDevice(h->device));
  cudaStream_t st = static_cast<cudaStream_t>(stream);
  rc = ensure_workspace(h, B, L);
  if (rc) return rc;
  {
    StageTimer tm(h, st, PCAD_ST_MISC);
    const long long n = static_cast<long long>(B) * L;
    ids64_to_u8_kernel<<<static_cast<unsigned>((n + 255) / 256), 256, 0, st>>>(reinterpret_cast<const long long*>(ids_dev), h->ws.ids, n, h->V, h->bad_flag);
    CUDA_TRY(h, cudaGetLastError());
  }
  rc = run_backbone(h, B, L, st);
  if (rc) return rc;
  if (logits_dev) {
    rc = run_head(h, B, L, nullptr, 0, logits_dev, st);
    if (rc) return rc;
  }
  if (hidden_dev) {
    StageTimer tm(h, st, PCAD_ST_MISC);
    const long long total = static_cast<long long>(B) * L * (2 * h->d / 8);
    const unsigned blocks = static_cast<unsigned>((total + 255) / 256);
    if (h->f32) hidden_tap_kernel<float><<<blocks, 256, 0, st>>>(static_cast<const float*>(h->ws.normed), static_cast<float*>(hidden_dev), B, L, h->d);
    else hidden_tap_kernel<bf16><<<blocks, 256, 0, st>>>(static_cast<const bf16*>(h->ws.normed), static_cast<bf16*>(hidden_dev), B, L, h->d);
    CUDA_TRY(h, cudaGetLastError());
  }
  return PCAD_OK;
}

int pcad_score_masked(pcad_handle* h, const uint8_t* ids_dev, const int32_t* pos_dev, int B, int L, int n_mask, float* logits4_dev, void* stream) {
  int rc = check_call(h, B, L);
  if (rc) return rc;
  if (B == 0 || L == 0 || n_mask == 0) return PCAD_OK;
  if (!ids_dev || !pos_dev || !logits4_dev || n_mask < 0) return fail(h, PCAD_ERR_INVALID, "null or negative argument");
  CUDA_TRY(h, cudaSetDevice(h->device));
  cudaStream_t st = static_cast<cudaStream_t>(stream);
  rc = ensure_workspace(h, B, L);
  if (rc) return rc;
  {
    StageTimer tm(h, st, PCAD_ST_MISC);
    const long long n = static_cast<long long>(B) * L;
    ids_u8_check_kernel<<<static_cast<unsigned>((n + 255) / 256), 256, 0, st>>>(ids_dev, h->ws.ids, n, h->V, h->bad_flag);
    CUDA_TRY(h, cudaGetLastError());
  }
  rc = run_backbone(h, B, L, st);
  if (rc) return rc;
  return run_head(h, B, L, pos_dev, n_mask, logits4_dev, st);
}

int pcad_score_masked_at(pcad_handle* h, const uint8_t* ids_dev, int token_idx, int B, int L, float* logits4_dev, void* stream) {
  int rc = check_call(h, B, L);
  if (rc) return rc;
  if (B == 0 || L == 0) return PCAD_OK;
  if (!ids_dev || !logits4_dev) return fail(h, PCAD_ERR_INVALID, "null argument");
  if (token_idx < 0 || token_idx >= L) return fail(h, PCAD_ERR_INVALID, "token_idx %d outside [0, %d)", token_idx, L);
  CUDA_TRY(h, cudaSetDevice(h->device));
  cudaStream_t st = static_cast<cudaStream_t>(stream);
  rc = ensure_workspace(h, B, L);
  if (rc) return rc;
  Workspace& ws = h->ws;
  {
    StageTimer tm(h, st, PCAD_ST_MISC, 3);
    const long long n = static_cast<long long>(B) * L;
    ids_u8_check_kernel<<<static_cast<unsigned>((n + 255) / 256), 256, 0, st>>>(ids_dev, ws.ids, n, h->V, h->bad_flag);
    fill_int_kernel<<<(B + 255) / 256, 256, 0, st>>>(ws.pos, B, token_idx);
    fill_int_kernel<<<(B + 255) / 256, 256, 0, st>>>(ws.pos0, B, 0);
    CUDA_TRY(h, cudaGetLastError());
  }
  const bool prune = h->prune_last && !h->m2 && h->cfg.n_layer > 0;
  rc = run_backbone(h, B, L, st, prune ? token_idx : -1);
  if (rc) return rc;
  if (prune && h->last_pruned) return run_head(h, B, 1, ws.pos0, 1, logits4_dev, st);
  return run_head(h, B, L, ws.pos, 1, logits4_dev, st);
}

int pcad_hidden_at(pcad_handle* h, const uint8_t* ids_dev, const int32_t* pos_dev, int B, int L, int n_pos, void* hidden_dev, void* stream) {
  int rc = check_call(h, B, L);
  if (rc) return rc;
  if (B == 0 || L == 0 || n_pos == 0) return PCAD_OK;
  if (!ids_dev || !pos_dev || !hidden_dev || n_pos < 0) return fail(h, PCAD_ERR_INVALID, "null or negative argument");
  CUDA_TRY(h, cudaSetDevice(h->device));
  cudaStream_t st = static_cast<cudaStream_t>(stream);
  rc = ensure_workspace(h, B, L);
  if (rc) return rc;
  {
    StageTimer tm(h, st, PCAD_ST_MISC);
    const long long n = static_cast<long long>(B) * L;
    ids_u8_check_kernel<<<static_cast<unsigned>((n + 255) / 256), 256, 0, st>>>(ids_dev, h->ws.ids, n, h->V, h->bad_flag);
    CUDA_TRY(h, cudaGetLastError());
  }
  rc = run_backbone(h, B, L, st);
  if (rc) return rc;
  StageTimer tm(h, st, PCAD_ST_MISC);
  const long long total = static_cast<long long>(B) * n_pos * (2 * h->d / 8);
  const unsigned blocks = static_cast<unsigned>((total + 255) / 256);
  if (h->f32) hidden_tap_pos_kernel<float><<<blocks, 256, 0, st>>>(static_cast<const float*>(h->ws.normed), pos_dev, n_pos, static_cast<float*>(hidden_dev), B, L, h->d);
  else hidden_tap_pos_kernel<bf16><<<blocks, 256, 0, st>>>(static_cast<const bf16*>(h->ws.normed), pos_dev, n_pos, static_cast<bf16*>(hidden_dev), B, L, h->d);
  CUDA_TRY(h, cudaGetLastError());
  return PCAD_OK;
}

int pcad_score_windows_host(pcad_handle* h, const uint8_t* ascii_host, int B, int L, int token_idx, float* logits4_host, void* stream) {
  int rc = check_call(h, B, L);
  if (rc) return rc;
  if (B == 0 || L == 0) return PCAD_OK;
  if (!ascii_host || !logits4_host) return fail(h, PCAD_ERR_INVALID, "null argument");
  if (token_idx < 0 || token_idx >= L) return fail(h, PCAD_ERR_INVALID, "token_idx %d outside [0, %d)", token_idx, L);
  CUDA_TRY(h, cudaSetDevice(h->device));
  cudaStream_t st = static_cast<cudaStream_t>(stream);
  rc = ensure_workspace(h, B, L);
  if (rc) return rc;
  Workspace& ws = h->ws;
  CUDA_TRY(h, cudaMemcpyAsync(ws.ascii, ascii_host, static_cast<size_t>(B) * L, cudaMemcpyHostToDevice, st));
  rc = score_core_graphed(h, B, L, token_idx, st);
  if (rc) return rc;
  CUDA_TRY(h, cudaMemcpyAsync(logits4_host, ws.logits4, static_cast<size_t>(B) * 4 * sizeof(float), cudaMemcpyDeviceToHost, st));
  CUDA_TRY(h, cudaStreamSynchronize(st));
  return PCAD_OK;
}

int pcad_take_id_error(pcad_handle* h, void* stream, int sync) {
  if (!h) return PCAD_ERR_INVALID;
  if (sync) {
    CUDA_TRY(h, cudaSetDevice(h->device));
    CUDA_TRY(h, cudaStreamSynchronize(static_cast<cudaStream_t>(stream)));
  }
  if (h->bad_flag_host && *h->bad_flag_host) {
    *h->bad_flag_host = 0;
    return fail(h, PCAD_ERR_INVALID, "token id outside [0, %d) in an earlier pcad_forward / pcad_score_masked call (the row was scored with id 0)", h->V);
  }
  return PCAD_OK;
}

int pcad_set_profiling(pcad_handle* h, int enabled) {
  if (!h) return PCAD_ERR_INVALID;
  for (auto& pe : h->prof_events) { h->event_pool.push_back(pe.second.first); h->event_pool.push_back(pe.second.second); }
  h->prof_events.clear();
  memset(h->prof_ms, 0, sizeof(h->prof_ms));
  memset(h->prof_launches, 0, sizeof(h->prof_launches));
  h->profiling = enabled != 0;
  return PCAD_OK;
}

int pcad_get_profile(pcad_handle* h, float ms[PCAD_ST_COUNT], int64_t launches[PCAD_ST_COUNT]) {
  if (!h || !ms || !launches) return PCAD_ERR_INVALID;
  CUDA_TRY(h, cudaSetDevice(h->device));
  for (auto& pe : h->prof_events) {
    CUDA_TRY(h, cudaEventSynchronize(pe.second.second));
    float t = 0.f;
    CUDA_TRY(h, cudaEventElapsedTime(&t, pe.second.first, pe.second.second));
    h->prof_ms[pe.first] += t;
    h->event_pool.push_back(pe.second.first);
    h->event_pool.push_back(pe.second.second);
  }
  h->prof_events.clear();
  for (int i = 0; i < PCAD_ST_COUNT; ++i) { ms[i] = h->prof_ms[i]; launches[i] = h->prof_launches[i]; }
  return PCAD_OK;
}

int64_t pcad_launch_count(const pcad_handle* h) { return h ? h->launch_count : 0; }

int pcad_op_sumsq_parts(int N) { return N > 0 ? gemm_sumsq_parts(N) : 0; }

static pcad_handle* op_scratch() {
  static pcad_handle scratch;
  return &scratch;
}
static int op_fail_to_global(int rc) {
  if (rc != PCAD_OK) snprintf(g_create_error, sizeof(g_create_error), "%.511s", op_scratch()->err);
  return rc;
}
static int op_num_sms() {
  int dev = 0, n = 148;
  cudaGetDevice(&dev);
  cudaDeviceGetAttribute(&n, cudaDevAttrMultiProcessorCount, dev);
  return n;
}

int pcad_op_linear(const void* A, const void* W, void* C, int64_t M, int N, int K, int64_t lda, int64_t ldw, int64_t ldc, int dtype, void* stream) {
  if (dtype != PCAD_BF16 && dtype != PCAD_F32) return PCAD_ERR_INVALID;
  return op_fail_to_global(op_linear(op_scratch(), A, W, C, M, N, K, lda, ldw, ldc, dtype == PCAD_F32, op_num_sms(), static_cast<cudaStream_t>(stream)));
}

int pcad_op_linear_residual(const void* A, const void* W, const void* resid_in, void* resid_out, float* sumsq_out, int64_t M, int N, int K,
                            int64_t lda, int64_t ldw, int64_t ld_res, int dtype, void* stream) {
  if (dtype != PCAD_BF16 || !resid_in || !sumsq_out) return PCAD_ERR_INVALID;
  EpiParams ep;
  ep.resid = static_cast<const bf16*>(resid_in);
  ep.ld_res = ld_res;
  ep.sumsq_out = sumsq_out;
  ep.sumsq_parts = gemm_sumsq_parts(N);
  return op_fail_to_global(op_linear(op_scratch(), A, W, resid_out, M, N, K, lda, ldw, ld_res, false, op_num_sms(), static_cast<cudaStream_t>(stream), kEpiResidual, ep));
}

int pcad_op_linear_rowscale(const void* A, const void* W, const float* sumsq_in, int sumsq_parts, float eps, void* C, int64_t M, int N, int K,
                            int64_t lda, int64_t ldw, int64_t ldc, int dtype, void* stream) {
  if (dtype != PCAD_BF16 || !sumsq_in || sumsq_parts < 1) return PCAD_ERR_INVALID;
  EpiParams ep;
  ep.sumsq_in = sumsq_in;
  ep.sumsq_parts = sumsq_parts;
  ep.inv_k = 1.0f / static_cast<float>(K);
  ep.eps = eps;
  return op_fail_to_global(op_linear(op_scratch(), A, W, C, M, N, K, lda, ldw, ldc, false, op_num_sms(), static_cast<cudaStream_t>(stream), kEpiRowScale, ep));
}

int pcad_op_biscan_dt(const void* u_f, const void* dbc_f, const void* u_r, const void* dbc_r, int64_t ldbc, int bc_off,
                      const void* wdt_f, const void* wdt_r, int64_t ldw, int R, const void* z, int64_t ldz, const float* A_f,
                      const float* D_f, const float* dt_bias_f, const float* A_r, const float* D_r, const float* dt_bias_r, void* y,
                      int S, int L, int E, void* stream) {
  if (!wdt_f || !wdt_r) return PCAD_ERR_INVALID;
  return op_fail_to_global(op_biscan(op_scratch(), u_f, dbc_f, dbc_f, u_r, dbc_r, dbc_r, ldbc, bc_off, z, ldz, A_f, D_f, dt_bias_f,
                                     A_r, D_r, dt_bias_r, y, S, L, E, false, static_cast<cudaStream_t>(stream), wdt_f, wdt_r, ldw, R));
}

int pcad_op_add_rmsnorm(const void* x, const void* res_in, const float* w, void* y, void* res_out, int64_t rows, int d, float eps, int dtype, int res_dtype, void* stream) {
  if (dtype != PCAD_BF16 && dtype != PCAD_F32) return PCAD_ERR_INVALID;
  if (dtype == PCAD_F32 && res_dtype != PCAD_F32) return PCAD_ERR_INVALID;
  return op_fail_to_global(op_add_rmsnorm(op_scratch(), x, res_in, w, y, res_out, rows, d, eps, dtype == PCAD_F32, res_dtype == PCAD_F32, static_cast<cudaStream_t>(stream)));
}

int pcad_op_conv_silu(const void* x, int64_t ldx, const float* w_f, const float* b_f, const float* w_r, const float* b_r, void* out_f, void* out_r, int S, int L, int E, int dtype, void* stream) {
  if (dtype != PCAD_BF16 && dtype != PCAD_F32) return PCAD_ERR_INVALID;
  return op_fail_to_global(op_conv(op_scratch(), x, ldx, w_f, b_f, w_r, b_r, out_f, out_r, S, L, E, dtype == PCAD_F32, static_cast<cudaStream_t>(stream)));
}

int pcad_op_biscan(const void* u_f, const void* delta_f, const void* bc_f, const void* u_r, const void* delta_r, const void* bc_r,
                   int64_t ldbc, int bc_off, const void* z, int64_t ldz, const float* A_f, const float* D_f, const float* dt_bias_f,
                   const float* A_r, const float* D_r, const float* dt_bias_r, void* y, int S, int L, int E, int dtype, void* stream) {
  if (dtype != PCAD_BF16 && dtype != PCAD_F32) return PCAD_ERR_INVALID;
  return op_fail_to_global(op_biscan(op_scratch(), u_f, delta_f, bc_f, u_r, delta_r, bc_r, ldbc, bc_off, z, ldz, A_f, D_f, dt_bias_f,
                                     A_r, D_r, dt_bias_r, y, S, L, E, dtype == PCAD_F32, static_cast<cudaStream_t>(stream)));
}

int pcad_op_biscan_segmented(const void* u_f, const void* delta_f, const void* bc_f, const void* u_r, const void* delta_r, const void* bc_r,
                             int64_t ldbc, int bc_off, const void* z, int64_t ldz, const float* A_f, const float* D_f, const float* dt_bias_f,
                             const float* A_r, const float* D_r, const float* dt_bias_r, void* y, int S, int L, int E, int segments,
                             float* seg_state, float* seg_sumd, int dtype, void* stream) {
  if (dtype != PCAD_BF16 && dtype != PCAD_F32) return PCAD_ERR_INVALID;
  return op_fail_to_global(op_biscan(op_scratch(), u_f, delta_f, bc_f, u_r, delta_r, bc_r, ldbc, bc_off, z, ldz, A_f, D_f, dt_bias_f,
                                     A_r, D_r, dt_bias_r, y, S, L, E, dtype == PCAD_F32, static_cast<cudaStream_t>(stream), nullptr,
                                     nullptr, 0, 0, segments, seg_state, seg_sumd));
}

int pcad_op_ssd_scan(const void* xbc_f, const void* xbc_r, int64_t ld_xbc, const void* dt_raw, int64_t ld_dt, const float* A_f,
                     const float* D_f, const float* dt_bias_f, const float* A_r, const float* D_r, const float* dt_bias_r, void* y_f,
                     void* y_r, int S, int L, int H, int dtype, int sequential, void* stream) {
  if (dtype != PCAD_BF16 && dtype != PCAD_F32) return PCAD_ERR_INVALID;
  return op_fail_to_global(op_ssd_scan(op_scratch(), xbc_f, xbc_r, ld_xbc, dt_raw, ld_dt, A_f, D_f, dt_bias_f, A_r, D_r, dt_bias_r, y_f,
                                       y_r, S, L, H, dtype == PCAD_F32, sequential, static_cast<cudaStream_t>(stream)));
}

int pcad_op_gated_norm_sum(const void* y_f, const void* y_r, const void* z, int64_t ldz, const float* w_f, const float* w_r, void* out,
                           int64_t rows, int E, float eps, int dtype, void* stream) {
  if (dtype != PCAD_BF16 && dtype != PCAD_F32) return PCAD_ERR_INVALID;
  return op_fail_to_global(op_gated_norm_sum(op_scratch(), y_f, y_r, z, ldz, w_f, w_r, out, rows, E, eps, dtype == PCAD_F32,
                                             static_cast<cudaStream_t>(stream)));
}

}
```

plantcaduceus_b200/csrc/scan.cuh:

```cuda
#pragma once

#include <stdlib.h>

#include "common.cuh"

namespace pcad {

#ifndef PCAD_SCAN_TC
#define PCAD_SCAN_TC 16
#endif
constexpr int kScanTC = PCAD_SCAN_TC;
#ifndef PCAD_SCAN_CH
#define PCAD_SCAN_CH 64
#endif
constexpr int kScanCH = PCAD_SCAN_CH;
constexpr int kScanSeg8 = kScanCH / 8;
constexpr int kScanThreads = 2 * kScanCH;
constexpr int kScanN = 16;
#ifndef PCAD_SCAN_SPPOLY
#define PCAD_SCAN_SPPOLY 7
#endif
#ifndef PCAD_SCAN_UNROLL
#define PCAD_SCAN_UNROLL 8
#endif
constexpr int kScanUnroll = PCAD_SCAN_UNROLL;
#ifndef PCAD_SCAN_MINBLOCKS64
#define PCAD_SCAN_MINBLOCKS64 4
#endif
#ifndef PCAD_SCAN_MINBLOCKS
#define PCAD_SCAN_MINBLOCKS 3
#endif

template <int V> struct IntTag { static constexpr int value = V; };

constexpr int kScanDtK = 64;
constexpr int kScanTmemCols = 64;

constexpr int kScanPlain = 0, kScanFusedDt = 1, kScanBcF32 = 2;
template <typename T, int MODE> struct ScanStage;
template <typename T>
struct ScanStage<T, kScanPlain> {
  T u[2][kScanTC][kScanCH];
  T d[2][kScanTC][kScanCH];
  T bc_raw[2][kScanTC][2 * kScanN];
};
template <typename T>
struct ScanStage<T, kScanFusedDt> {
  T dt[2][kScanTC][kScanDtK];
  T u[2][kScanTC][kScanCH];
};
template <typename T>
struct ScanStage<T, kScanBcF32> {
  T u[2][kScanTC][kScanCH];
  T d[2][kScanTC][kScanCH];
  float bc[2][kScanTC][2 * kScanN];
};

template <typename T, int MODE> struct ScanShared;
template <typename T>
struct ScanShared<T, kScanPlain> {
  ScanStage<T, kScanPlain> st[2];
  float bc[2][kScanTC][2 * kScanN];
  T pz[2][2][kScanTC][kScanCH];
};
template <typename T>
struct ScanShared<T, kScanFusedDt> {
  T wdt[2][kScanCH][kScanDtK];
  ScanStage<T, kScanFusedDt> st[2];
  T bc_raw[2][kScanTC][2 * kScanN];
  float bc[2][kScanTC][2 * kScanN];
  T pz[2][2][kScanTC][kScanCH];
};
template <typename T>
struct ScanShared<T, kScanBcF32> {
  ScanStage<T, kScanBcF32> st[2];
  T pz[2][2][kScanTC][kScanCH];
};

template <bool PRECISE> struct ScanDir;

template <> struct ScanDir<true> {
  float h[kScanN], a[kScanN];
  float bias;
  __device__ __forceinline__ void init(const float* A, float bias_) {
    bias = bias_;
#pragma unroll
    for (int n = 0; n < kScanN; ++n) { h[n] = 0.f; a[n] = A ? A[n] : 0.f; }
  }
  static __device__ __forceinline__ float b_scale() { return 1.0f; }
  __device__ __forceinline__ void load_state(const float* p) {
#pragma unroll
    for (int n = 0; n < kScanN; ++n) h[n] = p[n];
  }
  __device__ __forceinline__ void store_state(float* p) const {
#pragma unroll
    for (int n = 0; n < kScanN; ++n) p[n] = h[n];
  }
  __device__ __forceinline__ float run_decay(float sd, int n) const { return expf(sd * a[n]); }
  __device__ __forceinline__ float delta(float raw) const { return softplus<true>(raw + bias); }
  __device__ __forceinline__ float step(float d, float du, float y0, const float* bc) {
    float y = y0;
#pragma unroll
    for (int n = 0; n < kScanN; ++n) {
      h[n] = fmaf(expf(d * a[n]), h[n], du * bc[n]);
      y = fmaf(h[n], bc[kScanN + n], y);
    }
    return y;
  }
};

template <> struct ScanDir<false> {
  f32x2 h[kScanN / 2], a[kScanN / 2];
  float bias_l2;
  __device__ __forceinline__ void init(const float* A, float bias_) {
    bias_l2 = bias_ * kLog2e;
#pragma unroll
    for (int p = 0; p < kScanN / 2; ++p) {
      h[p] = pack2(0.f, 0.f);
      a[p] = A ? pack2(A[2 * p], A[2 * p + 1]) : pack2(0.f, 0.f);
    }
  }
  static __device__ __forceinline__ float b_scale() { return kLn2; }
  __device__ __forceinline__ void load_state(const float* p) {
#pragma unroll
    for (int q = 0; q < kScanN / 2; ++q) h[q] = pack2(p[2 * q], p[2 * q + 1]);
  }
  __device__ __forceinline__ void store_state(float* p) const {
#pragma unroll
    for (int q = 0; q < kScanN / 2; ++q) unpack2(h[q], p[2 * q], p[2 * q + 1]);
  }
  __device__ __forceinline__ float run_decay(float sd, int n) const {
    float a0, a1;
    unpack2(a[n >> 1], a0, a1);
    return ex2_approx(sd * ((n & 1) ? a1 : a0));
  }
  __device__ __forceinline__ float delta(float raw) const {
    const float xl = fmaf(raw, kLog2e, bias_l2);
#if PCAD_SCAN_SPPOLY
    const float e = ex2_approx(-fabsf(xl));
#if PCAD_SCAN_SPPOLY >= 7
    float q = fmaf(2.035518363e-02f, e, -9.567064047e-02f);
    q = fmaf(q, e, 2.151583284e-01f);
    q = fmaf(q, e, -3.390359282e-01f);
    q = fmaf(q, e, 4.776608944e-01f);
    q = fmaf(q, e, -7.211598754e-01f);
    q = fmaf(q, e, 1.442693233e+00f);
#else
    float q = fmaf(-3.443166614e-02f, e, 1.460243315e-01f);
    q = fmaf(q, e, -3.030317128e-01f);
    q = fmaf(q, e, 4.691744745e-01f);
    q = fmaf(q, e, -7.204267383e-01f);
    q = fmaf(q, e, 1.442682981e+00f);
#endif
    return fmaf(q, e, fmaxf(xl, 0.0f));
#else
    const float sp = lg2_approx(1.0f + ex2_approx(xl));
    return xl > 20.0f * kLog2e ? xl : sp;
#endif
  }
  __device__ __forceinline__ float step(float d, float du, float y0, const float* bc) {
    const f32x2 dd = pack2(d, d), duu = pack2(du, du);
    const ulonglong2* bc2 = reinterpret_cast<const ulonglong2*>(bc);
    f32x2 acc[2] = {pack2(y0, 0.f), pack2(0.f, 0.f)};
#pragma unroll
    for (int g = 0; g < kScanN / 4; ++g) {
      const ulonglong2 Bq = bc2[g], Cq = bc2[kScanN / 4 + g];
      const f32x2 Bp[2] = {Bq.x, Bq.y}, Cp[2] = {Cq.x, Cq.y};
#pragma unroll
      for (int k = 0; k < 2; ++k) {
        const int p = 2 * g + k;
        float x0, x1;
        unpack2(mul2(dd, a[p]), x0, x1);
        const f32x2 dA = pack2(ex2_approx(x0), ex2_approx(x1));
        h[p] = fma2(dA, h[p], mul2(duu, Bp[k]));
        acc[k] = fma2(h[p], Cp[k], acc[k]);
      }
    }
    float s0, s1;
    unpack2(add2(acc[0], acc[1]), s0, s1);
    return s0 + s1;
  }
};

template <typename T, bool PRECISE, int MODE>
__global__ void __launch_bounds__(kScanThreads, PRECISE ? 1 : (kScanCH == 64 ? PCAD_SCAN_MINBLOCKS64 : PCAD_SCAN_MINBLOCKS))
biscan_kernel(const __grid_constant__ CUtensorMap tm_uf, const __grid_constant__ CUtensorMap tm_df,
              const __grid_constant__ CUtensorMap tm_bcf, const __grid_constant__ CUtensorMap tm_ur,
              const __grid_constant__ CUtensorMap tm_dr, const __grid_constant__ CUtensorMap tm_bcr,
              const __grid_constant__ CUtensorMap tm_wf, const __grid_constant__ CUtensorMap tm_wr, int dt_ksteps,
              const T* __restrict__ z, long long ldz, const float* __restrict__ A_f, const float* __restrict__ D_f,
              const float* __restrict__ bias_f, const float* __restrict__ A_r, const float* __restrict__ D_r,
              const float* __restrict__ bias_r, T* y, int L, int E, const float* __restrict__ h0, int Lrun) {
  constexpr bool FUSEDT = MODE == kScanFusedDt, BCF32 = MODE == kScanBcF32;
  static_assert(MODE == kScanPlain || (sizeof(T) == 2 && !PRECISE && kScanCH == 64 && kScanTC == 16),
                "the in-kernel dt_proj and the fp32 B|C rows are bf16-path features of the 64-channel, 16-step kernel");
  extern __shared__ __align__(1024) uint8_t scan_smem_raw[];
  typedef ScanShared<T, MODE> Shared;
  typedef ScanStage<T, MODE> Stage;
  Shared& sm = *reinterpret_cast<Shared*>(scan_smem_raw);
  __shared__ __align__(16) float ys_all[BCF32 ? 2 : 1][2][kScanTC][kScanCH];
  __shared__ __align__(8) uint64_t full_bar[2];
  __shared__ __align__(8) uint64_t dt_bar[2];
  __shared__ __align__(8) uint64_t w_bar;
  __shared__ uint32_t tmem_slot;

  const int tid = threadIdx.x;
  const int dir = tid / kScanCH;
  const int ch = tid & (kScanCH - 1);
  const int e0 = blockIdx.x * kScanCH;
  const int e = e0 + ch;
  const bool active = e < E;
  const int seq = blockIdx.y;
  const long long row0 = static_cast<long long>(seq) * L;
  const int nch = (Lrun + kScanTC - 1) / kScanTC;
  constexpr int VEC = 16 / sizeof(T);
  constexpr int SEGS = kScanCH / VEC;
  constexpr uint32_t kDtBytes = sizeof(T) * 2 * kScanTC * kScanDtK;
  constexpr uint32_t kStageBytes = FUSEDT ? sizeof(Stage) - kDtBytes + sizeof(T) * 2 * kScanTC * 2 * kScanN : sizeof(Stage);

  if (tid == 0) {
    mbar_init(&full_bar[0], FUSEDT ? 2 : 1);
    mbar_init(&full_bar[1], FUSEDT ? 2 : 1);
    if constexpr (FUSEDT) {
      if (smem_u32(scan_smem_raw) & 1023u) __trap();
      mbar_init(&dt_bar[0], 1);
      mbar_init(&dt_bar[1], 1);
      mbar_init(&w_bar, 1);
      tma_prefetch_desc(&tm_wf); tma_prefetch_desc(&tm_wr);
    }
    fence_mbar_init();
    tma_prefetch_desc(&tm_uf); tma_prefetch_desc(&tm_df); tma_prefetch_desc(&tm_bcf);
    tma_prefetch_desc(&tm_ur); tma_prefetch_desc(&tm_dr); tma_prefetch_desc(&tm_bcr);
  }
  uint32_t tmem = 0;
  if constexpr (FUSEDT) {
    if (tid < 32) {
      tmem_alloc<kScanTmemCols>(&tmem_slot);
      tmem_relinquish();
    }
    tc_fence_before();
    __syncthreads();
    tc_fence_after();
    tmem = tmem_slot;
  } else {
    __syncthreads();
  }

  auto issue = [&](int c, int stage) {
    Stage& s = sm.st[stage];
    uint64_t* bar = &full_bar[stage];
    mbar_arrive_expect_tx(bar, kStageBytes);
    const int rf = c * kScanTC, rr = L - (c + 1) * kScanTC;
    tma_load_3d(&s.u[0][0][0], &tm_uf, bar, e0, rf, seq);
    tma_load_3d(&s.u[1][0][0], &tm_ur, bar, e0, rr, seq);
    if constexpr (FUSEDT) {
      tma_load_3d(&sm.bc_raw[0][0][0], &tm_bcf, bar, 0, rf, seq);
      tma_load_3d(&sm.bc_raw[1][0][0], &tm_bcr, bar, 0, rr, seq);
      mbar_arrive_expect_tx(&dt_bar[stage], kDtBytes);
      tma_load_3d(&s.dt[0][0][0], &tm_df, &dt_bar[stage], 0, rf, seq);
      tma_load_3d(&s.dt[1][0][0], &tm_dr, &dt_bar[stage], 0, rr, seq);
    } else {
      if constexpr (BCF32) {
        tma_load_3d(&s.bc[0][0][0], &tm_bcf, bar, 0, rf, seq);
        tma_load_3d(&s.bc[1][0][0], &tm_bcr, bar, 0, rr, seq);
      } else {
        tma_load_3d(&s.bc_raw[0][0][0], &tm_bcf, bar, 0, rf, seq);
        tma_load_3d(&s.bc_raw[1][0][0], &tm_bcr, bar, 0, rr, seq);
      }
      tma_load_3d(&s.d[0][0][0], &tm_df, bar, e0, rf, seq);
      tma_load_3d(&s.d[1][0][0], &tm_dr, bar, e0, rr, seq);
    }
  };
  auto issue_dt_mma = [&](int c, int stage) {
    if constexpr (FUSEDT) {
      mbar_wait_or_trap(&dt_bar[stage], (c >> 1) & 1);
      tc_fence_after();
      constexpr uint32_t idesc = make_idesc_bf16(128, 2 * kScanTC);
      const uint64_t da = make_smem_desc_sw128(smem_u32(&sm.wdt[0][0][0]));
      const uint64_t db = make_smem_desc_sw128(smem_u32(&sm.st[stage].dt[0][0][0]));
      umma_bf16_ss_k64_commit(tmem + stage * 2 * kScanTC, da, db, idesc, dt_ksteps, &full_bar[stage]);
    }
  };

  ScanDir<PRECISE> S;
  {
    const float* A = dir ? A_r : A_f;
    const float* bias = dir ? bias_r : bias_f;
    S.init(active ? A + e * kScanN : nullptr, active ? bias[e] : 0.f);
    if (h0 != nullptr && active) S.load_state(h0 + ((static_cast<long long>(blockIdx.y) * 2 + dir) * E + e) * kScanN);
  }
  const float Dskip = active ? (dir ? D_r : D_f)[e] : 0.f;
  const float bscale = ScanDir<PRECISE>::b_scale();

  if (tid < 32 && elect_one()) {
    if constexpr (FUSEDT) {
      mbar_arrive_expect_tx(&w_bar, sizeof(sm.wdt));
      tma_load_3d(&sm.wdt[0][0][0], &tm_wf, &w_bar, 0, e0, 0);
      tma_load_3d(&sm.wdt[1][0][0], &tm_wr, &w_bar, 0, e0, 0);
    }
    issue(0, 0);
    if constexpr (FUSEDT) {
      mbar_wait_or_trap(&w_bar, 0);
      issue_dt_mma(0, 0);
    }
  }
  if constexpr (FUSEDT) mbar_wait_or_trap(&w_bar, 0);
  bool prev_late = false;
  for (int c = 0; c < nch; ++c) {
    const int stage = c & 1;
    const bool tma_warp = tid < 32, mma_warp = (tid >> 5) == 2;
    if constexpr (!FUSEDT) {
      if (tma_warp && c + 1 < nch) {
        if (elect_one()) issue(c + 1, stage ^ 1);
      }
    }
    const Stage& s = sm.st[stage];
    const int i0 = c * kScanTC;
    const int nsteps = min(kScanTC, Lrun - i0);
    const bool has_final = (L - 1 - (i0 + nsteps - 1)) < i0 + nsteps;
    if constexpr (MODE != kScanPlain) mbar_wait_or_trap(&full_bar[stage], (c >> 1) & 1);
    else mbar_wait(&full_bar[stage], (c >> 1) & 1);
    float (*ys)[kScanTC][kScanCH] = ys_all[BCF32 ? (c & 1) : 0];
    const bool late_chunk = (L - 1 - i0) < i0;
    if constexpr (!BCF32) {
#pragma unroll
      for (int gi = tid; gi < 2 * kScanTC * 2 * kScanN / 4; gi += kScanThreads) {
        const int dd = gi >> 7, r = gi & 127;
        const int j = r >> 3, k0 = (r & 7) * 4;
        const T* src;
        if constexpr (FUSEDT) src = &sm.bc_raw[dd][dd ? kScanTC - 1 - j : j][k0];
        else src = &s.bc_raw[dd][dd ? kScanTC - 1 - j : j][k0];
        float4 v;
        if constexpr (sizeof(T) == 2) {
          const uint2 raw = *reinterpret_cast<const uint2*>(src);
          v.x = __uint_as_float(raw.x << 16); v.y = __uint_as_float(raw.x & 0xffff0000u);
          v.z = __uint_as_float(raw.y << 16); v.w = __uint_as_float(raw.y & 0xffff0000u);
        } else {
          v = *reinterpret_cast<const float4*>(src);
        }
        if (k0 < kScanN) { v.x *= bscale; v.y *= bscale; v.z *= bscale; v.w *= bscale; }
        *reinterpret_cast<float4*>(&sm.bc[dd][j][k0]) = v;
      }
      __syncthreads();
      if constexpr (FUSEDT) {
        if (tma_warp && c + 1 < nch) {
          if (elect_one()) issue(c + 1, stage ^ 1);
        }
      }
    } else {
      if (has_final && !prev_late) __syncthreads();
      prev_late = late_chunk;
    }
    if (sizeof(T) == 2 && late_chunk) {
      const int j = tid / kScanSeg8, seg = tid % kScanSeg8;
      const int chn = e0 + seg * 8;
      if (j < nsteps && chn < E) {
        const long long rf = row0 + i0 + j, rr = row0 + (L - 1 - i0 - j);
        cp_async16(&sm.pz[0][0][j][seg * 8], y + rf * E + chn, 16);
        cp_async16(&sm.pz[1][0][j][seg * 8], z + rf * ldz + chn, 16);
        cp_async16(&sm.pz[0][1][j][seg * 8], y + rr * E + chn, 16);
        cp_async16(&sm.pz[1][1][j][seg * 8], z + rr * ldz + chn, 16);
      }
    } else if (has_final) {
      for (int idx = tid; idx < 2 * kScanTC * SEGS; idx += kScanThreads) {
        const int dd = idx / (kScanTC * SEGS);
        const int rem = idx - dd * (kScanTC * SEGS);
        const int j = rem / SEGS, seg = rem % SEGS;
        const int i = i0 + j, io = L - 1 - i;
        const int chn = e0 + seg * VEC;
        const bool ok = (j < nsteps) && (chn < E) && (io < i0 + nsteps);
        const long long r = row0 + (ok ? (dd ? io : i) : 0);
        const int chs = ok ? chn : 0;
        if (ok && io < i0) cp_async16(&sm.pz[0][dd][j][seg * VEC], y + r * E + chs, 16);
        if (ok) cp_async16(&sm.pz[1][dd][j][seg * VEC], z + r * ldz + chs, 16);
      }
    }
    cp_async_commit();

    if constexpr (FUSEDT) tc_fence_after();
    if (active || FUSEDT) {
      const float* bcp;
      if constexpr (BCF32) bcp = &s.bc[dir][0][0];
      else bcp = &sm.bc[dir][0][0];
      float* ysp = &ys[dir][0][ch];
      auto run_chunk = [&](auto rev_tag) {
        constexpr bool REV = decltype(rev_tag)::value != 0;
        const T* up = &s.u[REV ? 1 : 0][0][ch];
        auto row = [](int j) { return (REV ? kScanTC - 1 - j : j) * kScanCH; };
        float uu = ActT<T>::to_f(up[row(0)]);
        float dl;
        auto advance = [&](int j, int jn, float draw_n) -> float {
          const float uu_n = ActT<T>::to_f(up[row(jn)]);
          const float dl_n = S.delta(draw_n);
          const float yv = S.step(dl, dl * uu, Dskip * uu, bcp + (BCF32 && REV ? kScanTC - 1 - j : j) * 2 * kScanN);
          uu = uu_n;
          dl = dl_n;
          return yv;
        };
        if constexpr (FUSEDT) {
          const uint32_t tmem_dl = tmem + (static_cast<uint32_t>((tid >> 5) * 32) << 16) + stage * 2 * kScanTC + (REV ? kScanTC : 0);
          uint32_t dp2[kScanTC / 2 + 1];
          {
            uint32_t dr[kScanTC];
            tmem_ld_32x32b_x16(tmem_dl, dr);
            tmem_ld_wait();
#pragma unroll
            for (int q = 0; q < kScanTC / 2; ++q) {
              const int c0 = REV ? kScanTC - 1 - 2 * q : 2 * q, c1 = REV ? kScanTC - 2 - 2 * q : 2 * q + 1;
              dp2[q] = pack_bf16x2(__uint_as_float(dr[c0]), __uint_as_float(dr[c1]));
            }
            dp2[kScanTC / 2] = 0u;
          }
          auto lo = [](uint32_t w) { return __uint_as_float(w << 16); };
          auto hi = [](uint32_t w) { return __uint_as_float(w & 0xffff0000u); };
          dl = S.delta(lo(dp2[0]));
          int j = 0;
          uint32_t w[kScanUnroll / 2 + 1];
#pragma unroll
          for (int q = 0; q <= kScanUnroll / 2; ++q) w[q] = dp2[q];
          static_assert(kScanUnroll == 8, "the window logic below is written for 8-step blocks");
#pragma unroll 1
          for (; j + kScanUnroll <= nsteps; j += kScanUnroll) {
            float yv[kScanUnroll];
#pragma unroll
            for (int k = 0; k < kScanUnroll; ++k) {
              const uint32_t wn = w[(k + 1) >> 1];
              yv[k] = advance(j + k, min(j + k + 1, kScanTC - 1), ((k + 1) & 1) ? hi(wn) : lo(wn));
            }
#pragma unroll
            for (int k = 0; k < kScanUnroll; ++k) ysp[(j + k) * kScanCH] = yv[k];
#pragma unroll
            for (int q = 0; q <= kScanUnroll / 2; ++q) w[q] = dp2[min(q + kScanUnroll / 2, kScanTC / 2)];
          }
#pragma unroll 1
          for (; j < nsteps; ++j) {
            const int jn = min(j + 1, kScanTC - 1);
            const uint32_t rn = tmem_ld_32x32b_x1(tmem_dl + (REV ? kScanTC - 1 - jn : jn));
            tmem_ld_wait();
            ysp[j * kScanCH] = advance(j, jn, lo(pack_bf16x2(__uint_as_float(rn), 0.f)));
          }
        } else {
          const T* dp = &s.d[REV ? 1 : 0][0][ch];
          dl = S.delta(ActT<T>::to_f(dp[row(0)]));
          int j = 0;
#pragma unroll 1
          for (; j + kScanUnroll <= nsteps; j += kScanUnroll) {
            float yv[kScanUnroll];
#pragma unroll
            for (int k = 0; k < kScanUnroll; ++k) {
              const int jn = min(j + k + 1, kScanTC - 1);
              yv[k] = advance(j + k, jn, ActT<T>::to_f(dp[row(jn)]));
            }
#pragma unroll
            for (int k = 0; k < kScanUnroll; ++k) ysp[(j + k) * kScanCH] = yv[k];
          }
#pragma unroll 1
          for (; j < nsteps; ++j) {
            const int jn = min(j + 1, kScanTC - 1);
            ysp[j * kScanCH] = advance(j, jn, ActT<T>::to_f(dp[row(jn)]));
          }
        }
      };
      if (dir) run_chunk(IntTag<1>());
      else run_chunk(IntTag<0>());
    }
    if constexpr (FUSEDT) {
      tc_fence_before();
      if (mma_warp && c + 1 < nch) {
        if (elect_one()) issue_dt_mma(c + 1, stage ^ 1);
      }
    }
    cp_async_wait<0>();
    __syncthreads();

    bool fast_done = false;
    if constexpr (!PRECISE && sizeof(T) == 2) {
      const bool early = !has_final, late = late_chunk;
      if (early || late) {
        fast_done = true;
        static_assert(kScanTC * kScanSeg8 == kScanThreads, "one item per thread and direction");
        const int j = tid / kScanSeg8, seg = tid % kScanSeg8;
        const int chn = e0 + seg * 8;
        if (j < nsteps && chn < E) {
#pragma unroll
          for (int dd = 0; dd < 2; ++dd) {
            const int i = i0 + j;
            const int t = dd ? L - 1 - i : i;
            const float4 a = *reinterpret_cast<const float4*>(&ys[dd][j][seg * 8]);
            const float4 b = *reinterpret_cast<const float4*>(&ys[dd][j][seg * 8 + 4]);
            f32x2 v2[4] = {pack2(a.x, a.y), pack2(a.z, a.w), pack2(b.x, b.y), pack2(b.z, b.w)};
            if (late) {
              const uint4 pr = *reinterpret_cast<const uint4*>(&sm.pz[0][dd][j][seg * 8]);
              const uint4 zr = *reinterpret_cast<const uint4*>(&sm.pz[1][dd][j][seg * 8]);
              const uint32_t pw[4] = {pr.x, pr.y, pr.z, pr.w}, zw[4] = {zr.x, zr.y, zr.z, zr.w};
              const f32x2 nl2 = pack2(-kLog2e, -kLog2e), one2 = pack2(1.0f, 1.0f);
#pragma unroll
              for (int q = 0; q < 4; ++q) {
                const f32x2 p2 = pack2(__uint_as_float(pw[q] << 16), __uint_as_float(pw[q] & 0xffff0000u));
                const f32x2 z2 = pack2(__uint_as_float(zw[q] << 16), __uint_as_float(zw[q] & 0xffff0000u));
                float x0, x1, d0, d1;
                unpack2(mul2(z2, nl2), x0, x1);
                unpack2(add2(pack2(ex2_approx(x0), ex2_approx(x1)), one2), d0, d1);
                const f32x2 g2 = mul2(z2, pack2(rcp_approx(d0), rcp_approx(d1)));
                v2[q] = mul2(add2(v2[q], p2), g2);
              }
            }
            uint4 out;
            float lo, hi;
            unpack2(v2[0], lo, hi); out.x = pack_bf16x2(lo, hi);
            unpack2(v2[1], lo, hi); out.y = pack_bf16x2(lo, hi);
            unpack2(v2[2], lo, hi); out.z = pack_bf16x2(lo, hi);
            unpack2(v2[3], lo, hi); out.w = pack_bf16x2(lo, hi);
            *reinterpret_cast<uint4*>(y + (row0 + t) * E + chn) = out;
          }
        }
      }
    }
    if (fast_done) continue;
    for (int idx = tid; idx < 2 * kScanTC * SEGS; idx += kScanThreads) {
      const int dd = idx / (kScanTC * SEGS);
      const int rem = idx - dd * (kScanTC * SEGS);
      const int j = rem / SEGS, seg = rem % SEGS;
      const int chn = e0 + seg * VEC;
      if (j >= nsteps || chn >= E) continue;
      const int i = i0 + j;
      const int io = L - 1 - i;
      const int t = dd ? io : i;
      float v[VEC];
#pragma unroll
      for (int k = 0; k < VEC; ++k) v[k] = ys[dd][j][seg * VEC + k];
      T* yp = y + (row0 + t) * E + chn;
      if (io >= i0 + nsteps) {
        store16<T>(yp, v);
        continue;
      }
      if (io >= i0) {
        if (io > i || (io == i && dd == 1)) continue;
#pragma unroll
        for (int k = 0; k < VEC; ++k) v[k] += ys[dd ^ 1][io - i0][seg * VEC + k];
      } else {
        float p[VEC];
        load16<T>(&sm.pz[0][dd][j][seg * VEC], p);
#pragma unroll
        for (int k = 0; k < VEC; ++k) v[k] += p[k];
      }
      float zz[VEC];
      load16<T>(&sm.pz[1][dd][j][seg * VEC], zz);
#pragma unroll
      for (int k = 0; k < VEC; ++k) v[k] *= silu<PRECISE>(zz[k]);
      store16<T>(yp, v);
    }
  }
  if constexpr (FUSEDT) {
    tc_fence_before();
    __syncthreads();
    if (tid < 32) tmem_dealloc<kScanTmemCols>(tmem);
  }
}

__global__ void bc_to_f32_kernel(const bf16* __restrict__ dbc_f, const bf16* __restrict__ dbc_r, long long ldbc, int bc_off,
                                 float* __restrict__ out, long long rows) {
  const long long idx = static_cast<long long>(blockIdx.x) * blockDim.x + threadIdx.x;
  if (idx >= rows * 8) return;
  const int q = static_cast<int>(idx & 3), dd = static_cast<int>((idx >> 2) & 1);
  const long long r = idx >> 3;
  const uint4 raw = *reinterpret_cast<const uint4*>((dd ? dbc_r : dbc_f) + r * ldbc + bc_off + 8 * q);
  const float sc = q < 2 ? kLn2 : 1.0f;
  const uint32_t w[4] = {raw.x, raw.y, raw.z, raw.w};
  float4 o0, o1;
  o0.x = __uint_as_float(w[0] << 16) * sc; o0.y = __uint_as_float(w[0] & 0xffff0000u) * sc;
  o0.z = __uint_as_float(w[1] << 16) * sc; o0.w = __uint_as_float(w[1] & 0xffff0000u) * sc;
  o1.x = __uint_as_float(w[2] << 16) * sc; o1.y = __uint_as_float(w[2] & 0xffff0000u) * sc;
  o1.z = __uint_as_float(w[3] << 16) * sc; o1.w = __uint_as_float(w[3] & 0xffff0000u) * sc;
  float4* op = reinterpret_cast<float4*>(out + (static_cast<long long>(dd) * rows + r) * 2 * kScanN + 8 * q);
  op[0] = o0;
  op[1] = o1;
}

template <typename T, bool PRECISE, int MODE = kScanPlain>
inline cudaError_t launch_biscan(const T* u_f, const T* delta_f, const T* bc_f, const T* u_r, const T* delta_r,
                                 const T* bc_r, long long ldbc, int bc_off, const T* z, long long ldz,
                                 const float* A_f, const float* D_f, const float* bias_f, const float* A_r,
                                 const float* D_r, const float* bias_r, T* y, int S, int L, int E,
                                 cudaStream_t stream, const T* wdt_f = nullptr, const T* wdt_r = nullptr, long long ldw = 0,
                                 int R = 0, const float* h0 = nullptr, int Lrun = 0, const float* bcf_f = nullptr,
                                 const float* bcf_r = nullptr) {
  constexpr bool FUSEDT = MODE == kScanFusedDt, BCF32 = MODE == kScanBcF32;
  size_t smem = sizeof(ScanShared<T, MODE>);
  if (const char* ex = getenv("PCAD_SCAN_EXTRA_SMEM")) smem += static_cast<size_t>(atoi(ex));
  static unsigned long long attr_done = 0;
  cudaError_t e1 = ensure_dynamic_smem(biscan_kernel<T, PRECISE, MODE>, static_cast<int>(smem), attr_done);
  if (e1 != cudaSuccess) return e1;
  constexpr bool f32 = sizeof(T) == 4;
  CUtensorMap tm[8];
  bool ok = make_tmap_3d(&tm[0], f32, u_f, E, L, S, E, kScanCH, kScanTC) && make_tmap_3d(&tm[2], f32, u_r, E, L, S, E, kScanCH, kScanTC);
  if (FUSEDT) {
    if (ldbc < kScanDtK || !wdt_f || !wdt_r || R <= 0 || R > kScanDtK || ldw < R || (ldw % 8)) return cudaErrorInvalidValue;
    ok = ok && make_tmap_3d(&tm[1], f32, delta_f, ldbc, L, S, ldbc, kScanDtK, kScanTC, true) &&
         make_tmap_3d(&tm[3], f32, delta_r, ldbc, L, S, ldbc, kScanDtK, kScanTC, true);
    ok = ok && make_tmap_3d(&tm[6], f32, wdt_f, R, E, 1, ldw, kScanDtK, kScanCH, true) &&
         make_tmap_3d(&tm[7], f32, wdt_r, R, E, 1, ldw, kScanDtK, kScanCH, true);
  } else {
    ok = ok && make_tmap_3d(&tm[1], f32, delta_f, E, L, S, E, kScanCH, kScanTC) &&
         make_tmap_3d(&tm[3], f32, delta_r, E, L, S, E, kScanCH, kScanTC);
    tm[6] = tm[0];
    tm[7] = tm[0];
  }
  if (BCF32) {
    if (!bcf_f || !bcf_r) return cudaErrorInvalidValue;
    ok = ok && make_tmap_3d(&tm[4], true, bcf_f, 2 * kScanN, L, S, 2 * kScanN, 2 * kScanN, kScanTC);
    ok = ok && make_tmap_3d(&tm[5], true, bcf_r, 2 * kScanN, L, S, 2 * kScanN, 2 * kScanN, kScanTC);
  } else {
    ok = ok && make_tmap_3d(&tm[4], f32, bc_f + bc_off, 2 * kScanN, L, S, ldbc, 2 * kScanN, kScanTC);
    ok = ok && make_tmap_3d(&tm[5], f32, bc_r + bc_off, 2 * kScanN, L, S, ldbc, 2 * kScanN, kScanTC);
  }
  if (!ok) return cudaErrorInvalidValue;
  dim3 grid((E + kScanCH - 1) / kScanCH, S);
  biscan_kernel<T, PRECISE, MODE><<<grid, kScanThreads, smem, stream>>>(
      tm[0], tm[1], tm[4], tm[2], tm[3], tm[5], tm[6], tm[7], (R + 15) / 16, z, ldz, A_f, D_f, bias_f, A_r, D_r, bias_r, y, L, E,
      h0, (Lrun > 0 && Lrun < L) ? Lrun : L);
  return cudaGetLastError();
}

template <typename T, bool PRECISE>
__global__ void __launch_bounds__(kScanThreads)
scan_segment_state_kernel(const T* __restrict__ u_f, const T* __restrict__ delta_f, const T* __restrict__ bc_f,
                          const T* __restrict__ u_r, const T* __restrict__ delta_r, const T* __restrict__ bc_r, long long ldbc,
                          int bc_off, const float* __restrict__ A_f, const float* __restrict__ bias_f,
                          const float* __restrict__ A_r, const float* __restrict__ bias_r, float* __restrict__ hend,
                          float* __restrict__ sumd, int Lseg, int E) {
  __shared__ __align__(16) float sbc[2][kScanTC][2 * kScanN];
  const int tid = threadIdx.x;
  const int dir = tid / kScanCH, ch = tid & (kScanCH - 1);
  const int e = blockIdx.x * kScanCH + ch;
  const bool active = e < E;
  const long long row0 = static_cast<long long>(blockIdx.y) * Lseg;
  const T* u = dir ? u_r : u_f;
  const T* dl = dir ? delta_r : delta_f;
  ScanDir<PRECISE> S;
  S.init(active ? (dir ? A_r : A_f) + e * kScanN : nullptr, active ? (dir ? bias_r : bias_f)[e] : 0.f);
  const float bscale = ScanDir<PRECISE>::b_scale();
  float sd = 0.f;
  for (int i0 = 0; i0 < Lseg; i0 += kScanTC) {
    const int nst = min(kScanTC, Lseg - i0);
    __syncthreads();
    for (int idx = tid; idx < 2 * kScanTC * 2 * kScanN; idx += kScanThreads) {
      const int dd = idx / (kScanTC * 2 * kScanN), rem = idx % (kScanTC * 2 * kScanN);
      const int j = rem / (2 * kScanN), k = rem % (2 * kScanN);
      float v = 0.f;
      if (j < nst) {
        const long long r = row0 + (dd ? Lseg - 1 - (i0 + j) : i0 + j);
        v = ActT<T>::to_f((dd ? bc_r : bc_f)[r * ldbc + bc_off + k]);
      }
      sbc[dd][j][k] = k < kScanN ? v * bscale : v;
    }
    float uu[kScanTC], dr[kScanTC];
#pragma unroll
    for (int j = 0; j < kScanTC; ++j) {
      const long long r = row0 + (dir ? Lseg - 1 - (i0 + j) : i0 + j);
      const bool ok = active && j < nst;
      uu[j] = ok ? ActT<T>::to_f(u[r * E + e]) : 0.f;
      dr[j] = ok ? ActT<T>::to_f(dl[r * E + e]) : 0.f;
    }
    __syncthreads();
    if (active) {
#pragma unroll
      for (int j = 0; j < kScanTC; ++j) {
        if (j < nst) {
          const float d = S.delta(dr[j]);
          sd += d;
          S.step(d, d * uu[j], 0.f, &sbc[dir][j][0]);
        }
      }
    }
  }
  if (active) {
    const long long o = (static_cast<long long>(blockIdx.y) * 2 + dir) * E + e;
    S.store_state(hend + o * kScanN);
    sumd[o] = sd;
  }
}

template <bool PRECISE>
__global__ void scan_segment_carry_kernel(const float* __restrict__ A_f, const float* __restrict__ A_r, float* __restrict__ hend,
                                          const float* __restrict__ sumd, int S, int P, int E) {
  const long long gid = static_cast<long long>(blockIdx.x) * blockDim.x + threadIdx.x;
  if (gid >= static_cast<long long>(S) * 2 * E) return;
  const int e = static_cast<int>(gid % E);
  const int dir = static_cast<int>((gid / E) % 2);
  const int seq = static_cast<int>(gid / (2LL * E));
  ScanDir<PRECISE> D;
  D.init((dir ? A_r : A_f) + e * kScanN, 0.f);
  float carry[kScanN];
#pragma unroll
  for (int n = 0; n < kScanN; ++n) carry[n] = 0.f;
  for (int k = 0; k < P; ++k) {
    const int seg = dir ? P - 1 - k : k;
    const long long o = ((static_cast<long long>(seq) * P + seg) * 2 + dir) * E + e;
    float* hp = hend + o * kScanN;
    const float sd = sumd[o];
#pragma unroll
    for (int n = 0; n < kScanN; ++n) {
      const float end0 = hp[n];
      hp[n] = carry[n];
      carry[n] = fmaf(D.run_decay(sd, n), carry[n], end0);
    }
  }
}

template <typename T, bool PRECISE>
inline cudaError_t launch_biscan_time_parallel(const T* u_f, const T* delta_f, const T* bc_f, const T* u_r, const T* delta_r,
                                               const T* bc_r, long long ldbc, int bc_off, const T* z, long long ldz,
                                               const float* A_f, const float* D_f, const float* bias_f, const float* A_r,
                                               const float* D_r, const float* bias_r, T* y, int S, int L, int E, int P,
                                               float* state, float* sumd, cudaStream_t stream, const float* bcf_f = nullptr,
                                               const float* bcf_r = nullptr) {
  if (P < 2 || L % P) return cudaErrorInvalidValue;
  const int Lseg = L / P;
  dim3 grid((E + kScanCH - 1) / kScanCH, S * P);
  scan_segment_state_kernel<T, PRECISE><<<grid, kScanThreads, 0, stream>>>(u_f, delta_f, bc_f, u_r, delta_r, bc_r, ldbc, bc_off, A_f,
                                                                           bias_f, A_r, bias_r, state, sumd, Lseg, E);
  const long long n = static_cast<long long>(S) * 2 * E;
  scan_segment_carry_kernel<PRECISE><<<static_cast<unsigned>((n + 127) / 128), 128, 0, stream>>>(A_f, A_r, state, sumd, S, P, E);
  cudaError_t e = cudaGetLastError();
  if (e != cudaSuccess) return e;
  if constexpr (sizeof(T) == 2 && !PRECISE) {
    if (bcf_f && bcf_r)
      return launch_biscan<T, PRECISE, kScanBcF32>(u_f, delta_f, bc_f, u_r, delta_r, bc_r, ldbc, bc_off, z, ldz, A_f, D_f, bias_f, A_r,
                                                   D_r, bias_r, y, S * P, Lseg, E, stream, nullptr, nullptr, 0, 0, state, 0, bcf_f, bcf_r);
  }
  return launch_biscan<T, PRECISE, kScanPlain>(u_f, delta_f, bc_f, u_r, delta_r, bc_r, ldbc, bc_off, z, ldz, A_f, D_f, bias_f, A_r, D_r,
                                               bias_r, y, S * P, Lseg, E, stream, nullptr, nullptr, 0, 0, state);
}

}
```

Before: 890.6.

## Enable fused dt_proj scan by default with TMEM-resident weights and fp32 B|C rows

The in-kernel dt_proj GEMM now keeps the dt_proj weights in tensor memory, loaded once per CTA with tcgen05.st, and issues the MMA with A taken from TMEM (ts form). This frees the shared-memory weight tile and the TMA weight load. The fused path now also consumes the pre-converted fp32 B|C rows, so the per-chunk bf16-to-fp32 conversion and its __syncthreads are gone. dt loads and MMAs are pipelined two chunks ahead on their own warps. The fused path is turned on by default for large token counts; it saves the separate dt_proj GEMM and the delta round trip through global memory, at the cost of a bc_to_f32 pass and a doubled TMEM allocation.

```diff
diff --git a/plantcaduceus_b200/csrc/common.cuh b/plantcaduceus_b200/csrc/common.cuh
--- a/plantcaduceus_b200/csrc/common.cuh
+++ b/plantcaduceus_b200/csrc/common.cuh
@@ -303,24 +303,24 @@
       "l"(desc_a), "l"(desc_b), "r"(idesc), "r"(accumulate)
       : "memory");
 }
-__device__ __forceinline__ void umma_bf16_ss_k64_commit(uint32_t tmem_d, uint64_t desc_a, uint64_t desc_b, uint32_t idesc,
+__device__ __forceinline__ void umma_bf16_ts_k64_commit(uint32_t tmem_d, uint32_t tmem_a, uint64_t desc_b, uint32_t idesc,
                                                         int ksteps, uint64_t* bar) {
   asm volatile(
-      "{\n\t.reg .pred pz, po, p1, p2, p3;\n\t.reg .b64 a1, b1, a2, b2, a3, b3;\n\t"
+      "{\n\t.reg .pred pz, po, p1, p2, p3;\n\t.reg .b32 a1, a2, a3;\n\t.reg .b64 b1, b2, b3;\n\t"
       "setp.ne.b32 pz, 0, 0;\n\t"
       "setp.eq.b32 po, 0, 0;\n\t"
       "setp.gt.s32 p1, %4, 1;\n\t"
       "setp.gt.s32 p2, %4, 2;\n\t"
       "setp.gt.s32 p3, %4, 3;\n\t"
-      "add.s64 a1, %1, 2;\n\tadd.s64 b1, %2, 2;\n\t"
-      "add.s64 a2, %1, 4;\n\tadd.s64 b2, %2, 4;\n\t"
-      "add.s64 a3, %1, 6;\n\tadd.s64 b3, %2, 6;\n\t"
-      "tcgen05.mma.cta_group::1.kind::f16 [%0], %1, %2, %3, pz;\n\t"
-      "@p1 tcgen05.mma.cta_group::1.kind::f16 [%0], a1, b1, %3, po;\n\t"
-      "@p2 tcgen05.mma.cta_group::1.kind::f16 [%0], a2, b2, %3, po;\n\t"
-      "@p3 tcgen05.mma.cta_group::1.kind::f16 [%0], a3, b3, %3, po;\n\t"
+      "add.u32 a1, %1, 8;\n\tadd.s64 b1, %2, 2;\n\t"
+      "add.u32 a2, %1, 16;\n\tadd.s64 b2, %2, 4;\n\t"
+      "add.u32 a3, %1, 24;\n\tadd.s64 b3, %2, 6;\n\t"
+      "tcgen05.mma.cta_group::1.kind::f16 [%0], [%1], %2, %3, pz;\n\t"
+      "@p1 tcgen05.mma.cta_group::1.kind::f16 [%0], [a1], b1, %3, po;\n\t"
+      "@p2 tcgen05.mma.cta_group::1.kind::f16 [%0], [a2], b2, %3, po;\n\t"
+      "@p3 tcgen05.mma.cta_group::1.kind::f16 [%0], [a3], b3, %3, po;\n\t"
       "tcgen05.commit.cta_group::1.mbarrier::arrive::one.shared::cluster.b64 [%5];\n\t}\n" ::"r"(tmem_d),
-      "l"(desc_a), "l"(desc_b), "r"(idesc), "r"(ksteps), "r"(smem_u32(bar))
+      "r"(tmem_a), "l"(desc_b), "r"(idesc), "r"(ksteps), "r"(smem_u32(bar))
       : "memory");
 }
 __device__ __forceinline__ void umma_commit(uint64_t* bar) {
@@ -354,6 +354,18 @@
   return r;
 }
 __device__ __forceinline__ void tmem_ld_wait() { asm volatile("tcgen05.wait::ld.sync.aligned;\n" ::: "memory"); }
+__device__ __forceinline__ void tmem_st_32x32b_x32(uint32_t taddr, const uint32_t (&r)[32]) {
+  asm volatile(
+      "tcgen05.st.sync.aligned.32x32b.x32.b32 [%0], "
+      "{%1, %2, %3, %4, %5, %6, %7, %8, %9, %10, %11, %12, %13, %14, %15, %16, "
+      "%17, %18, %19, %20, %21, %22, %23, %24, %25, %26, %27, %28, %29, %30, %31, %32};\n" ::"r"(taddr),
+      "r"(r[0]), "r"(r[1]), "r"(r[2]), "r"(r[3]), "r"(r[4]), "r"(r[5]), "r"(r[6]), "r"(r[7]), "r"(r[8]), "r"(r[9]),
+      "r"(r[10]), "r"(r[11]), "r"(r[12]), "r"(r[13]), "r"(r[14]), "r"(r[15]), "r"(r[16]), "r"(r[17]), "r"(r[18]),
+      "r"(r[19]), "r"(r[20]), "r"(r[21]), "r"(r[22]), "r"(r[23]), "r"(r[24]), "r"(r[25]), "r"(r[26]), "r"(r[27]),
+      "r"(r[28]), "r"(r[29]), "r"(r[30]), "r"(r[31])
+      : "memory");
+}
+__device__ __forceinline__ void tmem_st_wait() { asm volatile("tcgen05.wait::st.sync.aligned;\n" ::: "memory"); }
 
 __device__ __forceinline__ uint32_t cluster_ctarank() {
   uint32_t r;
diff --git a/plantcaduceus_b200/csrc/pcad.cu b/plantcaduceus_b200/csrc/pcad.cu
--- a/plantcaduceus_b200/csrc/pcad.cu
+++ b/plantcaduceus_b200/csrc/pcad.cu
@@ -79,6 +79,7 @@
   int H = 0, CD = 0, DIP = 0, DIPP = 0;
   bool f32 = false;
   bool fuse_dt = false;
+  bool fuse_dt_force = false;
   bool bc_f32 = true;
   bool bc_f32_force = false;
   bool fuse_norm = false;
@@ -326,9 +327,12 @@
       static_cast<const TT*>(delta_r), static_cast<const TT*>(bc_r), ldbc, bc_off, static_cast<const TT*>(z), ldz, A_f, D_f, \
       bias_f, A_r, D_r, bias_r, static_cast<TT*>(y), S, L, E
   const bool fused_dt = wdt_f != nullptr || wdt_r != nullptr;
+  if (fused_dt && (f32 || !bcf || !wdt_f || !wdt_r || ldbc < kScanDtK || R <= 0 || R > kScanDtK || ldw < R || ldw % 8))
+    return fail(h, PCAD_ERR_INVALID, "biscan: the in-kernel dt_proj needs bf16, the fp32 B|C scratch, both weights (R <= 64, row pitch "
+                "a multiple of 8) and ldbc >= 64");
   const float* bcf_f = nullptr;
   const float* bcf_r = nullptr;
-  if (bcf && !f32 && !fused_dt) {
+  if (bcf && !f32) {
     const long long rows = static_cast<long long>(S) * L;
     bc_to_f32_kernel<<<static_cast<unsigned>((rows * 8 + 255) / 256), 256, 0, st>>>(static_cast<const bf16*>(bc_f), static_cast<const bf16*>(bc_r),
                                                                                   ldbc, bc_off, bcf, rows);
@@ -345,10 +349,8 @@
     return PCAD_OK;
   }
   if (fused_dt) {
-    if (f32 || !wdt_f || !wdt_r || ldbc < kScanDtK || R <= 0 || R > kScanDtK || ldw < R || ldw % 8)
-      return fail(h, PCAD_ERR_INVALID, "biscan: the in-kernel dt_proj needs bf16, both weights (R <= 64, row pitch a multiple of 8) and ldbc >= 64");
     e = launch_biscan<bf16, false, kScanFusedDt>(PCAD_SCAN_ARGS(bf16), st, static_cast<const bf16*>(wdt_f), static_cast<const bf16*>(wdt_r),
-                                                 ldw, R, nullptr, Lrun);
+                                                 ldw, R, nullptr, Lrun, bcf_f, bcf_r);
   } else if (f32) {
     e = launch_biscan<float, true, kScanPlain>(PCAD_SCAN_ARGS(float), st, nullptr, nullptr, 0, 0, nullptr, Lrun);
   } else if (bcf_f) {
@@ -363,6 +365,7 @@
 
 size_t align_up(size_t v, size_t a) { return (v + a - 1) / a * a; }
 constexpr size_t kSegStateBytes = 16u << 20;
+constexpr long long kFuseDtMinTokens = 32768;
 
 size_t workspace_layout(const pcad_handle* h, int B, int L, Workspace* ws) {
   const size_t T = 2ull * B * L;
@@ -574,7 +577,7 @@
              static_cast<size_t>(S) * P * 2 * 2 * E * kScanN * sizeof(float) <= kSegStateBytes)
         P *= 2;
     }
-    const bool fuse_dt = h->fuse_dt && P == 1;
+    const bool fuse_dt = h->fuse_dt && P == 1 && (h->fuse_dt_force || T >= kFuseDtMinTokens);
     for (int dir = 0; dir < 2; ++dir) {
       {
         StageTimer tm(h, st, PCAD_ST_X_PROJ);
@@ -593,11 +596,12 @@
       pruned = prune_idx >= 0 && li == h->cfg.n_layer - 1 && P == 1 && h->prune_last && L >= 8;
       const int Lrun = pruned ? (prune_idx > L - 1 - prune_idx ? prune_idx : L - 1 - prune_idx) + 1 : 0;
       const bool use_bcf = h->bc_f32 && !f32 && (h->bc_f32_force || T >= 65536);
-      if (fuse_dt)
+      if (fuse_dt) {
         rc = op_biscan(h, ws.xc[0], ws.dbc[0], ws.dbc[0], ws.xc[1], ws.dbc[1], ws.dbc[1], RP, R, zbase, 2 * E,
                        lw.dir[0].A, lw.dir[0].D, lw.dir[0].dt_bias, lw.dir[1].A, lw.dir[1].D, lw.dir[1].dt_bias, ws.y, S, L, E, f32,
-                       st, lw.dir[0].dt_proj, lw.dir[1].dt_proj, R, R, 1, nullptr, nullptr, Lrun);
-      else {
+                       st, lw.dir[0].dt_proj, lw.dir[1].dt_proj, R, R, 1, nullptr, nullptr, Lrun, ws.bcf);
+        h->launch_count += 1;
+      } else {
         rc = op_biscan(h, ws.xc[0], ws.delta[0], ws.dbc[0], ws.xc[1], ws.delta[1], ws.dbc[1], RP, R, zbase, 2 * E,
                        lw.dir[0].A, lw.dir[0].D, lw.dir[0].dt_bias, lw.dir[1].A, lw.dir[1].D, lw.dir[1].dt_bias, ws.y, S, L, E, f32, st,
                        nullptr, nullptr, 0, 0, P, ws.seg_state, ws.seg_sumd, Lrun, use_bcf ? ws.bcf : nullptr);
@@ -759,9 +763,8 @@
   h->f32 = cfg->dtype == PCAD_F32;
   h->act_size = h->f32 ? 4 : 2;
   h->fuse_norm = !h->f32 && !cfg->residual_in_fp32;
-  h->fuse_dt = false;
-  if (const char* fd = getenv("PCAD_FUSED_DT"))
-    h->fuse_dt = fd[0] == '1' && !m2 && !h->f32 && h->RP >= kScanDtK && h->R <= kScanDtK && (h->E % 8) == 0;
+  h->fuse_dt = !m2 && !h->f32 && h->RP >= kScanDtK && h->R <= kScanDtK && (h->R % 8) == 0;
+  if (const char* fd = getenv("PCAD_FUSED_DT")) { h->fuse_dt = h->fuse_dt && fd[0] != '0'; h->fuse_dt_force = fd[0] == '1'; }
   if (const char* bq = getenv("PCAD_SCAN_BC_F32")) { h->bc_f32 = bq[0] != '0'; h->bc_f32_force = bq[0] == '1'; }
   if (const char* pl = getenv("PCAD_NO_PRUNE")) h->prune_last = pl[0] != '1';
   if (const char* tp = getenv("PCAD_NO_TIME_PARALLEL")) h->time_parallel = tp[0] != '1';
@@ -1339,8 +1342,16 @@
                       const float* D_f, const float* dt_bias_f, const float* A_r, const float* D_r, const float* dt_bias_r, void* y,
                       int S, int L, int E, void* stream) {
   if (!wdt_f || !wdt_r) return PCAD_ERR_INVALID;
-  return op_fail_to_global(op_biscan(op_scratch(), u_f, dbc_f, dbc_f, u_r, dbc_r, dbc_r, ldbc, bc_off, z, ldz, A_f, D_f, dt_bias_f,
-                                     A_r, D_r, dt_bias_r, y, S, L, E, false, static_cast<cudaStream_t>(stream), wdt_f, wdt_r, ldw, R));
+  const cudaStream_t st = static_cast<cudaStream_t>(stream);
+  float* bcf = nullptr;
+  if (S > 0 && L > 0) {
+    const cudaError_t ea = cudaMallocAsync(reinterpret_cast<void**>(&bcf), static_cast<size_t>(S) * L * 2 * 2 * kScanN * sizeof(float), st);
+    if (ea != cudaSuccess) return op_fail_to_global(fail(op_scratch(), PCAD_ERR_CUDA, "biscan_dt: %s", cudaGetErrorString(ea)));
+  }
+  const int rc = op_biscan(op_scratch(), u_f, dbc_f, dbc_f, u_r, dbc_r, dbc_r, ldbc, bc_off, z, ldz, A_f, D_f, dt_bias_f, A_r, D_r,
+                           dt_bias_r, y, S, L, E, false, st, wdt_f, wdt_r, ldw, R, 1, nullptr, nullptr, 0, bcf);
+  if (bcf) cudaFreeAsync(bcf, st);
+  return op_fail_to_global(rc);
 }
 
 int pcad_op_add_rmsnorm(const void* x, const void* res_in, const float* w, void* y, void* res_out, int64_t rows, int d, float eps, int dtype, int res_dtype, void* stream) {
diff --git a/plantcaduceus_b200/csrc/scan.cuh b/plantcaduceus_b200/csrc/scan.cuh
--- a/plantcaduceus_b200/csrc/scan.cuh
+++ b/plantcaduceus_b200/csrc/scan.cuh
@@ -34,7 +34,7 @@
 template <int V> struct IntTag { static constexpr int value = V; };
 
 constexpr int kScanDtK = 64;
-constexpr int kScanTmemCols = 64;
+constexpr int kScanTmemCols = 128, kScanTmemW = 0, kScanTmemDelta = 32;
 
 constexpr int kScanPlain = 0, kScanFusedDt = 1, kScanBcF32 = 2;
 template <typename T, int MODE> struct ScanStage;
@@ -46,8 +46,8 @@
 };
 template <typename T>
 struct ScanStage<T, kScanFusedDt> {
-  T dt[2][kScanTC][kScanDtK];
   T u[2][kScanTC][kScanCH];
+  float bc[2][kScanTC][2 * kScanN];
 };
 template <typename T>
 struct ScanStage<T, kScanBcF32> {
@@ -65,10 +65,8 @@
 };
 template <typename T>
 struct ScanShared<T, kScanFusedDt> {
-  T wdt[2][kScanCH][kScanDtK];
+  T dt[2][2][kScanTC][kScanDtK];
   ScanStage<T, kScanFusedDt> st[2];
-  T bc_raw[2][kScanTC][2 * kScanN];
-  float bc[2][kScanTC][2 * kScanN];
   T pz[2][2][kScanTC][kScanCH];
 };
 template <typename T>
@@ -187,21 +185,21 @@
 biscan_kernel(const __grid_constant__ CUtensorMap tm_uf, const __grid_constant__ CUtensorMap tm_df,
               const __grid_constant__ CUtensorMap tm_bcf, const __grid_constant__ CUtensorMap tm_ur,
               const __grid_constant__ CUtensorMap tm_dr, const __grid_constant__ CUtensorMap tm_bcr,
-              const __grid_constant__ CUtensorMap tm_wf, const __grid_constant__ CUtensorMap tm_wr, int dt_ksteps,
+              const T* __restrict__ wdt_f, const T* __restrict__ wdt_r, long long ldw, int R,
               const T* __restrict__ z, long long ldz, const float* __restrict__ A_f, const float* __restrict__ D_f,
               const float* __restrict__ bias_f, const float* __restrict__ A_r, const float* __restrict__ D_r,
               const float* __restrict__ bias_r, T* y, int L, int E, const float* __restrict__ h0, int Lrun) {
-  constexpr bool FUSEDT = MODE == kScanFusedDt, BCF32 = MODE == kScanBcF32;
+  constexpr bool FUSEDT = MODE == kScanFusedDt;
+  constexpr bool ROWS32 = MODE != kScanPlain;
   static_assert(MODE == kScanPlain || (sizeof(T) == 2 && !PRECISE && kScanCH == 64 && kScanTC == 16),
                 "the in-kernel dt_proj and the fp32 B|C rows are bf16-path features of the 64-channel, 16-step kernel");
   extern __shared__ __align__(1024) uint8_t scan_smem_raw[];
   typedef ScanShared<T, MODE> Shared;
   typedef ScanStage<T, MODE> Stage;
   Shared& sm = *reinterpret_cast<Shared*>(scan_smem_raw);
-  __shared__ __align__(16) float ys_all[BCF32 ? 2 : 1][2][kScanTC][kScanCH];
+  __shared__ __align__(16) float ys_all[ROWS32 ? 2 : 1][2][kScanTC][kScanCH];
   __shared__ __align__(8) uint64_t full_bar[2];
   __shared__ __align__(8) uint64_t dt_bar[2];
-  __shared__ __align__(8) uint64_t w_bar;
   __shared__ uint32_t tmem_slot;
 
   const int tid = threadIdx.x;
@@ -216,7 +214,6 @@
   constexpr int VEC = 16 / sizeof(T);
   constexpr int SEGS = kScanCH / VEC;
   constexpr uint32_t kDtBytes = sizeof(T) * 2 * kScanTC * kScanDtK;
-  constexpr uint32_t kStageBytes = FUSEDT ? sizeof(Stage) - kDtBytes + sizeof(T) * 2 * kScanTC * 2 * kScanN : sizeof(Stage);
 
   if (tid == 0) {
     mbar_init(&full_bar[0], FUSEDT ? 2 : 1);
@@ -225,8 +222,6 @@
       if (smem_u32(scan_smem_raw) & 1023u) __trap();
       mbar_init(&dt_bar[0], 1);
       mbar_init(&dt_bar[1], 1);
-      mbar_init(&w_bar, 1);
-      tma_prefetch_desc(&tm_wf); tma_prefetch_desc(&tm_wr);
     }
     fence_mbar_init();
     tma_prefetch_desc(&tm_uf); tma_prefetch_desc(&tm_df); tma_prefetch_desc(&tm_bcf);
@@ -242,6 +237,24 @@
     __syncthreads();
     tc_fence_after();
     tmem = tmem_slot;
+    uint32_t wr[kScanDtK / 2];
+    const T* wrow = (dir ? wdt_r : wdt_f) + static_cast<long long>(active ? e : 0) * ldw;
+#pragma unroll
+    for (int q = 0; q < kScanDtK / 8; ++q) {
+      uint4 v = make_uint4(0u, 0u, 0u, 0u);
+      if (active && 8 * q < R) v = *reinterpret_cast<const uint4*>(wrow + 8 * q);
+      wr[4 * q] = v.x; wr[4 * q + 1] = v.y; wr[4 * q + 2] = v.z; wr[4 * q + 3] = v.w;
+    }
+#pragma unroll
+    for (int k = 0; k < kScanDtK / 2; ++k) {
+      if (2 * k >= R) wr[k] = 0u;
+      else if (2 * k + 1 >= R) wr[k] &= 0xffffu;
+    }
+    tmem_st_32x32b_x32(tmem + (static_cast<uint32_t>((tid >> 5) * 32) << 16) + kScanTmemW, wr);
+    tmem_st_wait();
+    tc_fence_before();
+    __syncthreads();
+    tc_fence_after();
   } else {
     __syncthreads();
   }
@@ -249,36 +262,38 @@
   auto issue = [&](int c, int stage) {
     Stage& s = sm.st[stage];
     uint64_t* bar = &full_bar[stage];
-    mbar_arrive_expect_tx(bar, kStageBytes);
+    mbar_arrive_expect_tx(bar, sizeof(Stage));
     const int rf = c * kScanTC, rr = L - (c + 1) * kScanTC;
     tma_load_3d(&s.u[0][0][0], &tm_uf, bar, e0, rf, seq);
     tma_load_3d(&s.u[1][0][0], &tm_ur, bar, e0, rr, seq);
-    if constexpr (FUSEDT) {
-      tma_load_3d(&sm.bc_raw[0][0][0], &tm_bcf, bar, 0, rf, seq);
-      tma_load_3d(&sm.bc_raw[1][0][0], &tm_bcr, bar, 0, rr, seq);
-      mbar_arrive_expect_tx(&dt_bar[stage], kDtBytes);
-      tma_load_3d(&s.dt[0][0][0], &tm_df, &dt_bar[stage], 0, rf, seq);
-      tma_load_3d(&s.dt[1][0][0], &tm_dr, &dt_bar[stage], 0, rr, seq);
+    if constexpr (ROWS32) {
+      tma_load_3d(&s.bc[0][0][0], &tm_bcf, bar, 0, rf, seq);
+      tma_load_3d(&s.bc[1][0][0], &tm_bcr, bar, 0, rr, seq);
     } else {
-      if constexpr (BCF32) {
-        tma_load_3d(&s.bc[0][0][0], &tm_bcf, bar, 0, rf, seq);
-        tma_load_3d(&s.bc[1][0][0], &tm_bcr, bar, 0, rr, seq);
-      } else {
-        tma_load_3d(&s.bc_raw[0][0][0], &tm_bcf, bar, 0, rf, seq);
-        tma_load_3d(&s.bc_raw[1][0][0], &tm_bcr, bar, 0, rr, seq);
-      }
+      tma_load_3d(&s.bc_raw[0][0][0], &tm_bcf, bar, 0, rf, seq);
+      tma_load_3d(&s.bc_raw[1][0][0], &tm_bcr, bar, 0, rr, seq);
+    }
+    if constexpr (!FUSEDT) {
       tma_load_3d(&s.d[0][0][0], &tm_df, bar, e0, rf, seq);
       tma_load_3d(&s.d[1][0][0], &tm_dr, bar, e0, rr, seq);
     }
   };
-  auto issue_dt_mma = [&](int c, int stage) {
+  auto issue_dt = [&](int c) {
     if constexpr (FUSEDT) {
-      mbar_wait_or_trap(&dt_bar[stage], (c >> 1) & 1);
+      uint64_t* bar = &dt_bar[c & 1];
+      mbar_arrive_expect_tx(bar, kDtBytes);
+      tma_load_3d(&sm.dt[c & 1][0][0][0], &tm_df, bar, 0, c * kScanTC, seq);
+      tma_load_3d(&sm.dt[c & 1][1][0][0], &tm_dr, bar, 0, L - (c + 1) * kScanTC, seq);
+    }
+  };
+  auto issue_dt_mma = [&](int c) {
+    if constexpr (FUSEDT) {
+      mbar_wait_or_trap(&dt_bar[c & 1], (c >> 1) & 1);
       tc_fence_after();
       constexpr uint32_t idesc = make_idesc_bf16(128, 2 * kScanTC);
-      const uint64_t da = make_smem_desc_sw128(smem_u32(&sm.wdt[0][0][0]));
-      const uint64_t db = make_smem_desc_sw128(smem_u32(&sm.st[stage].dt[0][0][0]));
-      umma_bf16_ss_k64_commit(tmem + stage * 2 * kScanTC, da, db, idesc, dt_ksteps, &full_bar[stage]);
+      const uint64_t db = make_smem_desc_sw128(smem_u32(&sm.dt[c & 1][0][0][0]));
+      umma_bf16_ts_k64_commit(tmem + kScanTmemDelta + (c & 1) * 2 * kScanTC, tmem + kScanTmemW, db, idesc, (R + 15) / 16,
+                              &full_bar[c & 1]);
     }
   };
 
@@ -292,26 +307,22 @@
   const float Dskip = active ? (dir ? D_r : D_f)[e] : 0.f;
   const float bscale = ScanDir<PRECISE>::b_scale();
 
-  if (tid < 32 && elect_one()) {
-    if constexpr (FUSEDT) {
-      mbar_arrive_expect_tx(&w_bar, sizeof(sm.wdt));
-      tma_load_3d(&sm.wdt[0][0][0], &tm_wf, &w_bar, 0, e0, 0);
-      tma_load_3d(&sm.wdt[1][0][0], &tm_wr, &w_bar, 0, e0, 0);
-    }
+  const bool tma_warp = tid < 32, mma_warp = (tid >> 5) == 2;
+  if (tma_warp && elect_one()) {
     issue(0, 0);
-    if constexpr (FUSEDT) {
-      mbar_wait_or_trap(&w_bar, 0);
-      issue_dt_mma(0, 0);
-    }
-  }
-  if constexpr (FUSEDT) mbar_wait_or_trap(&w_bar, 0);
+    issue_dt(0);
+    if (nch > 1) issue_dt(1);
+  }
+  if (FUSEDT && mma_warp && elect_one()) issue_dt_mma(0);
   bool prev_late = false;
   for (int c = 0; c < nch; ++c) {
     const int stage = c & 1;
-    const bool tma_warp = tid < 32, mma_warp = (tid >> 5) == 2;
-    if constexpr (!FUSEDT) {
-      if (tma_warp && c + 1 < nch) {
-        if (elect_one()) issue(c + 1, stage ^ 1);
+    if (tma_warp && c + 1 < nch) {
+      if (elect_one()) issue(c + 1, stage ^ 1);
+    }
+    if constexpr (FUSEDT) {
+      if (mma_warp && c + 1 < nch) {
+        if (elect_one()) issue_dt_mma(c + 1);
       }
     }
     const Stage& s = sm.st[stage];
@@ -320,16 +331,19 @@
     const bool has_final = (L - 1 - (i0 + nsteps - 1)) < i0 + nsteps;
     if constexpr (MODE != kScanPlain) mbar_wait_or_trap(&full_bar[stage], (c >> 1) & 1);
     else mbar_wait(&full_bar[stage], (c >> 1) & 1);
-    float (*ys)[kScanTC][kScanCH] = ys_all[BCF32 ? (c & 1) : 0];
+    if constexpr (FUSEDT) {
+      if (tma_warp && c + 2 < nch) {
+        if (elect_one()) issue_dt(c + 2);
+      }
+    }
+    float (*ys)[kScanTC][kScanCH] = ys_all[ROWS32 ? (c & 1) : 0];
     const bool late_chunk = (L - 1 - i0) < i0;
-    if constexpr (!BCF32) {
+    if constexpr (!ROWS32) {
 #pragma unroll
       for (int gi = tid; gi < 2 * kScanTC * 2 * kScanN / 4; gi += kScanThreads) {
         const int dd = gi >> 7, r = gi & 127;
         const int j = r >> 3, k0 = (r & 7) * 4;
-        const T* src;
-        if constexpr (FUSEDT) src = &sm.bc_raw[dd][dd ? kScanTC - 1 - j : j][k0];
-        else src = &s.bc_raw[dd][dd ? kScanTC - 1 - j : j][k0];
+        const T* src = &s.bc_raw[dd][dd ? kScanTC - 1 - j : j][k0];
         float4 v;
         if constexpr (sizeof(T) == 2) {
           const uint2 raw = *reinterpret_cast<const uint2*>(src);
@@ -342,11 +356,6 @@
         *reinterpret_cast<float4*>(&sm.bc[dd][j][k0]) = v;
       }
       __syncthreads();
-      if constexpr (FUSEDT) {
-        if (tma_warp && c + 1 < nch) {
-          if (elect_one()) issue(c + 1, stage ^ 1);
-        }
-      }
     } else {
       if (has_final && !prev_late) __syncthreads();
       prev_late = late_chunk;
@@ -380,7 +389,7 @@
     if constexpr (FUSEDT) tc_fence_after();
     if (active || FUSEDT) {
       const float* bcp;
-      if constexpr (BCF32) bcp = &s.bc[dir][0][0];
+      if constexpr (ROWS32) bcp = &s.bc[dir][0][0];
       else bcp = &sm.bc[dir][0][0];
       float* ysp = &ys[dir][0][ch];
       auto run_chunk = [&](auto rev_tag) {
@@ -392,13 +401,14 @@
         auto advance = [&](int j, int jn, float draw_n) -> float {
           const float uu_n = ActT<T>::to_f(up[row(jn)]);
           const float dl_n = S.delta(draw_n);
-          const float yv = S.step(dl, dl * uu, Dskip * uu, bcp + (BCF32 && REV ? kScanTC - 1 - j : j) * 2 * kScanN);
+          const float yv = S.step(dl, dl * uu, Dskip * uu, bcp + (ROWS32 && REV ? kScanTC - 1 - j : j) * 2 * kScanN);
           uu = uu_n;
           dl = dl_n;
           return yv;
         };
         if constexpr (FUSEDT) {
-          const uint32_t tmem_dl = tmem + (static_cast<uint32_t>((tid >> 5) * 32) << 16) + stage * 2 * kScanTC + (REV ? kScanTC : 0);
+          const uint32_t tmem_dl =
+              tmem + (static_cast<uint32_t>((tid >> 5) * 32) << 16) + kScanTmemDelta + stage * 2 * kScanTC + (REV ? kScanTC : 0);
           uint32_t dp2[kScanTC / 2 + 1];
           {
             uint32_t dr[kScanTC];
@@ -464,12 +474,7 @@
       if (dir) run_chunk(IntTag<1>());
       else run_chunk(IntTag<0>());
     }
-    if constexpr (FUSEDT) {
-      tc_fence_before();
-      if (mma_warp && c + 1 < nch) {
-        if (elect_one()) issue_dt_mma(c + 1, stage ^ 1);
-      }
-    }
+    if constexpr (FUSEDT) tc_fence_before();
     cp_async_wait<0>();
     __syncthreads();
 
@@ -585,28 +590,26 @@
                                  cudaStream_t stream, const T* wdt_f = nullptr, const T* wdt_r = nullptr, long long ldw = 0,
                                  int R = 0, const float* h0 = nullptr, int Lrun = 0, const float* bcf_f = nullptr,
                                  const float* bcf_r = nullptr) {
-  constexpr bool FUSEDT = MODE == kScanFusedDt, BCF32 = MODE == kScanBcF32;
+  constexpr bool FUSEDT = MODE == kScanFusedDt, ROWS32 = MODE != kScanPlain;
   size_t smem = sizeof(ScanShared<T, MODE>);
   if (const char* ex = getenv("PCAD_SCAN_EXTRA_SMEM")) smem += static_cast<size_t>(atoi(ex));
   static unsigned long long attr_done = 0;
   cudaError_t e1 = ensure_dynamic_smem(biscan_kernel<T, PRECISE, MODE>, static_cast<int>(smem), attr_done);
   if (e1 != cudaSuccess) return e1;
   constexpr bool f32 = sizeof(T) == 4;
-  CUtensorMap tm[8];
+  CUtensorMap tm[6];
   bool ok = make_tmap_3d(&tm[0], f32, u_f, E, L, S, E, kScanCH, kScanTC) && make_tmap_3d(&tm[2], f32, u_r, E, L, S, E, kScanCH, kScanTC);
   if (FUSEDT) {
-    if (ldbc < kScanDtK || !wdt_f || !wdt_r || R <= 0 || R > kScanDtK || ldw < R || (ldw % 8)) return cudaErrorInvalidValue;
+    if (ldbc < kScanDtK || !wdt_f || !wdt_r || R <= 0 || R > kScanDtK || ldw < R || (ldw % 8) ||
+        ((reinterpret_cast<uintptr_t>(wdt_f) | reinterpret_cast<uintptr_t>(wdt_r)) & 15))
+      return cudaErrorInvalidValue;
     ok = ok && make_tmap_3d(&tm[1], f32, delta_f, ldbc, L, S, ldbc, kScanDtK, kScanTC, true) &&
          make_tmap_3d(&tm[3], f32, delta_r, ldbc, L, S, ldbc, kScanDtK, kScanTC, true);
-    ok = ok && make_tmap_3d(&tm[6], f32, wdt_f, R, E, 1, ldw, kScanDtK, kScanCH, true) &&
-         make_tmap_3d(&tm[7], f32, wdt_r, R, E, 1, ldw, kScanDtK, kScanCH, true);
   } else {
     ok = ok && make_tmap_3d(&tm[1], f32, delta_f, E, L, S, E, kScanCH, kScanTC) &&
          make_tmap_3d(&tm[3], f32, delta_r, E, L, S, E, kScanCH, kScanTC);
-    tm[6] = tm[0];
-    tm[7] = tm[0];
-  }
-  if (BCF32) {
+  }
+  if (ROWS32) {
     if (!bcf_f || !bcf_r) return cudaErrorInvalidValue;
     ok = ok && make_tmap_3d(&tm[4], true, bcf_f, 2 * kScanN, L, S, 2 * kScanN, 2 * kScanN, kScanTC);
     ok = ok && make_tmap_3d(&tm[5], true, bcf_r, 2 * kScanN, L, S, 2 * kScanN, 2 * kScanN, kScanTC);
@@ -617,7 +620,7 @@
   if (!ok) return cudaErrorInvalidValue;
   dim3 grid((E + kScanCH - 1) / kScanCH, S);
   biscan_kernel<T, PRECISE, MODE><<<grid, kScanThreads, smem, stream>>>(
-      tm[0], tm[1], tm[4], tm[2], tm[3], tm[5], tm[6], tm[7], (R + 15) / 16, z, ldz, A_f, D_f, bias_f, A_r, D_r, bias_r, y, L, E,
+      tm[0], tm[1], tm[4], tm[2], tm[3], tm[5], wdt_f, wdt_r, ldw, R, z, ldz, A_f, D_f, bias_f, A_r, D_r, bias_r, y, L, E,
       h0, (Lrun > 0 && Lrun < L) ? Lrun : L);
   return cudaGetLastError();
 }
```

Result: no change. 896.1 (median of 6 runs) (+0.6%).
